# argumentcomputer/lurk-beta

Measured on AMD Instinct MI355X. Metric: MSM Mscalar-mul/s (Pallas Pedersen commitment, bases+scalars resident in HBM), higher is better.
Workload: dtype u32x8 (255-bit Montgomery, integer VALU)

## Files before the change

### lurk_beta_amd/csrc/common.hpp

```cpp
#pragma once
#include <hip/hip_runtime.h>

#include <cstdint>
#include <cstdio>
#include <cstring>
#include <condition_variable>
#include <functional>
#include <map>
#include <mutex>
#include <string>
#include <thread>
#include <utility>
#include <vector>

#include "../../include/lurk_hip.h"

namespace lurk {

void set_error(int code, const std::string& msg);
int last_error_code();

struct HipFailure {
    int code;
    std::string msg;
};

#define LURK_HIP_CHECK(expr)                                                                              \
    do {                                                                                                  \
        hipError_t _e = (expr);                                                                           \
        if (_e != hipSuccess) {                                                                           \
            (void)hipGetLastError();  \
            throw ::lurk::HipFailure{_e == hipErrorOutOfMemory ? LURK_HIP_ERR_OOM : LURK_HIP_ERR_HIP,     \
                                     std::string(#expr) + ": " + hipGetErrorString(_e)};                 \
        }                                                                                                 \
    } while (0)

#define LURK_REQUIRE(cond, msg)                                                       \
    do {                                                                              \
        if (!(cond)) throw ::lurk::HipFailure{LURK_HIP_ERR_INVALID_ARG, std::string(msg)}; \
    } while (0)

void require_device();

struct DeviceGuard {
    int prev = -1;
    bool switched = false;
    explicit DeviceGuard(int dev) {
        LURK_HIP_CHECK(hipGetDevice(&prev));
        if (prev != dev) {
            LURK_HIP_CHECK(hipSetDevice(dev));
            switched = true;
        }
    }
    ~DeviceGuard() {
        if (switched) (void)hipSetDevice(prev);
    }
    DeviceGuard(const DeviceGuard&) = delete;
    DeviceGuard& operator=(const DeviceGuard&) = delete;
};
int current_device();

void allow_dynamic_lds(const void* kernel, int bytes);

template <class F>
int host_guarded(F&& f) {
    try {
        f();
        set_error(0, "");
        return 0;
    } catch (const HipFailure& e) {
        set_error(e.code, e.msg);
        return e.code;
    } catch (const std::exception& e) {
        set_error(LURK_HIP_ERR_HIP, e.what());
        return LURK_HIP_ERR_HIP;
    }
}
template <class F>
int guarded(F&& f) {
    return host_guarded([&] {
        require_device();
        f();
    });
}
inline void nested_ok(int rc) {
    if (rc != 0) throw HipFailure{rc, lurk_hip_last_error()};
}

struct DevBuf {
    void* p = nullptr;
    size_t bytes = 0;
    DevBuf() = default;
    explicit DevBuf(size_t n) { alloc(n); }
    DevBuf(const DevBuf&) = delete;
    DevBuf& operator=(const DevBuf&) = delete;
    DevBuf(DevBuf&& o) noexcept : p(o.p), bytes(o.bytes) { o.p = nullptr; o.bytes = 0; }
    DevBuf& operator=(DevBuf&& o) noexcept {
        if (this != &o) { release(); p = o.p; bytes = o.bytes; o.p = nullptr; o.bytes = 0; }
        return *this;
    }
    ~DevBuf() { release(); }
    void alloc(size_t n) {
        release();
        if (n == 0) n = 16;
        LURK_HIP_CHECK(hipMalloc(&p, n));
        bytes = n;
    }
    void ensure(size_t n) {
        if (n > bytes) alloc(n);
    }
    void release() {
        if (p) (void)hipFree(p);
        p = nullptr;
        bytes = 0;
    }
    template <class T>
    T* as() const { return reinterpret_cast<T*>(p); }
};

class Profiler {
  public:
    static Profiler& get();
    void enable(bool on) { enabled_ = on; }
    bool enabled() const { return enabled_; }
    void reset();
    hipEvent_t begin(hipStream_t s);
    void end(const char* name, hipEvent_t a, hipStream_t s);
    void query(const char* prefix, double* total_ms, uint64_t* launches);

  private:
    struct Rec { std::string name; hipEvent_t a, b; int device; hipStream_t s; };
    std::mutex mu_;
    bool enabled_ = false;
    std::vector<Rec> recs_;
    std::map<int, std::vector<hipEvent_t>> pool_;
    std::map<std::string, std::pair<double, uint64_t>> done_;
    hipEvent_t get_event(int device);
    void dump_timeline();
};

struct ProfScope {
    hipStream_t s;
    const char* name;
    hipEvent_t a = nullptr;
    ProfScope(const char* nm, hipStream_t st) : s(st), name(nm) {
        if (Profiler::get().enabled()) a = Profiler::get().begin(s);
    }
    ~ProfScope() {
        if (a) Profiler::get().end(name, a, s);
    }
};

class DeviceWorker {
  public:
    explicit DeviceWorker(int device);
    ~DeviceWorker();
    void post(std::function<void()> job);
    void wait();
    int device() const { return device_; }

  private:
    void loop();
    int device_;
    std::mutex mu_;
    std::condition_variable cv_;
    std::function<void()> job_;
    bool has_job_ = false, busy_ = false, stop_ = false, failed_ = false;
    HipFailure err_{0, ""};
    std::thread th_;
};

struct MsmTableView {
    const void* table = nullptr;
    size_t npoints = 0;
    int curve = 0, window_bits = 0, windows = 1, form = 0, device = 0;
};
MsmTableView msm_ctx_table_view(const lurk_hip_msm_ctx* ctx);
int msm_multi_curve(const lurk_hip_msm_multi* key);
void msm_ctx_wait_pair_xyzz(lurk_hip_msm_ctx* ctx, int slot, void* out_lo_xyzz128, void* out_hi_xyzz128);
struct FoldedKeyLease {
    lurk_hip_msm_ctx* ctx = nullptr;
    bool owned = false;
    std::unique_lock<std::mutex> lk;
    FoldedKeyLease() = default;
    FoldedKeyLease(FoldedKeyLease&& o) noexcept : ctx(o.ctx), owned(o.owned), lk(std::move(o.lk)) {
        o.ctx = nullptr;
        o.owned = false;
    }
    FoldedKeyLease(const FoldedKeyLease&) = delete;
    ~FoldedKeyLease();
};
FoldedKeyLease msm_ctx_folded_child(lurk_hip_msm_ctx* parent, const void* d_points, size_t m, hipStream_t s);
void msm_ctx_drop_folded_child(const lurk_hip_msm_ctx* parent);

class ScratchArena {
  public:
    static ScratchArena& of(hipStream_t s);
    static size_t trim_all();
    void* push(size_t bytes);
    void pop(void* p);
    std::recursive_mutex mu;

  private:
    struct Block { char* base; size_t cap, top; };
    struct Live { void* p; size_t block, prev_top; bool freed; };
    std::vector<Block> blocks_;
    std::vector<Live> live_;
    size_t cur_ = 0;
};
struct ArenaBuf {
    ScratchArena* arena;
    void* p = nullptr;
    ArenaBuf(size_t bytes, hipStream_t s) : arena(&ScratchArena::of(s)) {
        arena->mu.lock();
        try {
            p = arena->push(bytes ? bytes : 32);
        } catch (...) {
            arena->mu.unlock();
            throw;
        }
    }
    ~ArenaBuf() {
        arena->pop(p);
        arena->mu.unlock();
    }
    ArenaBuf(const ArenaBuf&) = delete;
    ArenaBuf& operator=(const ArenaBuf&) = delete;
};

struct PoseidonImageView {
    const void* img = nullptr;
    int vec4 = 0, rf = 0, rp = 0;
};
PoseidonImageView poseidon_image_view(int field_id, int arity, hipStream_t s);

inline const char* curve_name(int curve) {
    switch (curve) {
        case LURK_CURVE_PALLAS: return "Pallas";
        case LURK_CURVE_VESTA: return "Vesta";
        case LURK_CURVE_BN254: return "BN254";
        case LURK_CURVE_GRUMPKIN: return "Grumpkin";
    }
    return "unknown";
}
inline void require_pasta_curve(int curve, const char* what) {
    if (curve == LURK_CURVE_PALLAS || curve == LURK_CURVE_VESTA) return;
    if (curve == LURK_CURVE_BN254 || curve == LURK_CURVE_GRUMPKIN)
        throw HipFailure{LURK_HIP_ERR_INVALID_ARG, std::string(what) + " is not offered on " + curve_name(curve) + " (Pallas and Vesta only)"};
    throw HipFailure{LURK_HIP_ERR_INVALID_ARG, "unknown curve id"};
}

inline unsigned div_up(size_t a, size_t b) { return (unsigned)((a + b - 1) / b); }

int num_cus();
unsigned grid_cap(unsigned per_cu);
void stream_pool_retain();

}
```

### lurk_beta_amd/csrc/curve29.cuh

```cuda
#pragma once
#include "curve.cuh"
#include "field29.cuh"

#ifndef LURK_ACC_Y3_ROW
#define LURK_ACC_Y3_ROW 1
#endif
#ifndef LURK_ACC_AFFINE_FIRST
#define LURK_ACC_AFFINE_FIRST 1
#endif
#ifndef LURK_F29_RARE_ATTR
#define LURK_F29_RARE_ATTR __attribute__((noinline))
#endif

namespace lurk {

template <class P>
LURK_HD F29<P> f29_carry_signed(const int32_t* t) {
    F29<P> r;
    int32_t c = 0;
#pragma unroll
    for (int i = 0; i < 8; i++) {
        int32_t x = t[i] + c;
        r.l[i] = (uint32_t)x & F29_MASK;
        c = x >> 29;
    }
    r.l[8] = (uint32_t)(t[8] + c);
    return r;
}


template <class P>
LURK_HD F29<P> f29_reduce_pasta(const F29<P>& v) {
    const uint32_t k = v.l[8] >> 22;
    const uint32_t km1 = k ? k - 1 : 0;
    int32_t t[9];
    uint64_t c = 0;
#pragma unroll
    for (int i = 0; i < 5; i++) {
        c += (uint64_t)km1 * f29_mod<P>(i);
        t[i] = (int32_t)v.l[i] - (int32_t)((uint32_t)c & F29_MASK);
        c >>= 29;
    }
    t[5] = (int32_t)v.l[5] - (int32_t)(uint32_t)c;
    t[6] = (int32_t)v.l[6];
    t[7] = (int32_t)v.l[7];
    t[8] = (int32_t)(v.l[8] & ((1u << 22) - 1u)) + (k ? (int32_t)(1u << 22) : 0);
    return f29_carry_signed<P>(t);
}
template <class P>
LURK_HD F29<P> f29_reduce_general(const F29<P>& v) {
    constexpr uint32_t D = (P::mod(7) >> 8) + 1u;
    static_assert(D > (1u << 21) && D <= (1u << 22), "f29_reduce_general: the modulus must have 253 or 254 bits");
    constexpr uint64_t mu = ((uint64_t)1 << 53) / D;
    F29_ASSERT(v.l[8] < (1u << 31), "f29_reduce: top limb >= 2^31");
    const uint32_t q = (uint32_t)(((uint64_t)v.l[8] * mu) >> 53);
    int32_t t[9];
    uint64_t c = 0;
#pragma unroll
    for (int i = 0; i < 8; i++) {
        c += (uint64_t)q * f29_mod<P>(i);
        t[i] = (int32_t)v.l[i] - (int32_t)((uint32_t)c & F29_MASK);
        c >>= 29;
    }
    c += (uint64_t)q * f29_mod<P>(8);
    t[8] = (int32_t)v.l[8] - (int32_t)(uint32_t)c;
    const F29<P> r = f29_carry_signed<P>(t);
    F29_ASSERT(r.l[8] < (1u << 24), "f29_reduce: result not below 2^256");
    return r;
}
template <class P>
LURK_HD F29<P> f29_reduce(const F29<P>& v) {
    if constexpr (f29_pasta_shape<P>()) return f29_reduce_pasta<P>(v);
    else return f29_reduce_general<P>(v);
}

template <class P>
struct Xyzz29 {
    F29<P> x, y, zz, zzz;
};

template <class P>
LURK_HD Xyzz<P> xyzz29_to_xyzz(const Xyzz29<P>& a, bool is_identity) {
    if (is_identity) return xyzz_identity<P>();
    Xyzz<P> r;
    r.x = f29_to_mont256<P>(a.x);
    r.y = f29_to_mont256<P>(a.y);
    r.zz = f29_to_mont256<P>(a.zz);
    r.zzz = f29_to_mont256<P>(a.zzz);
    return r;
}
template <class P>
LURK_HD void xyzz29_from_xyzz(const Xyzz<P>& a, Xyzz29<P>& r, bool& is_identity) {
    is_identity = xyzz_is_identity<P>(a);
    r.x = f29_from_mont256<P>(a.x);
    r.y = f29_from_mont256<P>(a.y);
    r.zz = f29_from_mont256<P>(a.zz);
    r.zzz = f29_from_mont256<P>(a.zzz);
}

template <class P>
LURK_HD uint32_t f29_multiple_candidate(const F29<P>& v) {
    if constexpr (f29_pasta_shape<P>()) return v.l[0];
    else return (v.l[0] * ((0u - f29_inv<P>()) & F29_MASK)) & F29_MASK;
}
template <class P>
LURK_HD bool f29_maybe_multiple_of_p(const F29<P>& v) {
    return f29_multiple_candidate<P>(v) < (f29_pasta_shape<P>() ? 128u : 256u);
}
template <class P>
LURK_HD bool f29_is_multiple_of_p(const F29<P>& v) {
    const uint32_t k = f29_multiple_candidate<P>(v);
    uint64_t c = 0;
    bool eq = true;
#pragma unroll
    for (int i = 0; i < 8; i++) {
        c += (uint64_t)k * f29_mod<P>(i);
        eq = eq && (v.l[i] == ((uint32_t)c & F29_MASK));
        c >>= 29;
    }
    c += (uint64_t)k * f29_mod<P>(8);
    return eq && (uint64_t)v.l[8] == c;
}

template <class P>
LURK_HD LURK_F29_RARE_ATTR Xyzz29<P> xyzz29_double_affine(F29<P> qx, F29<P> qy_signed) {
    const F29<P> u = f29_dbl<P>(qy_signed);
    const F29<P> v = f29_mul<P>(u, u);
    const F29<P> w = f29_mul30<P>(u, v);
    const F29<P> s = f29_mul30<P>(qx, v);
    const F29<P> xx = f29_sqr30<P>(qx);
    const F29<P> m = f29_carry<P>(f29_add<P>(f29_dbl<P>(xx), xx));
    const F29<P> m2 = f29_sqr30<P>(m);
    Xyzz29<P> r;
    r.x = f29_reduce<P>(f29_carry<P>(f29_sub<P>(m2, f29_dbl<P>(s))));
    const F29<P> t1 = f29_mul<P>(m, f29_sub<P>(s, r.x));
    const F29<P> t2 = f29_mul30<P>(w, qy_signed);
    r.y = f29_reduce<P>(f29_carry<P>(f29_sub<P>(t1, t2)));
    r.zz = v;
    r.zzz = w;
    return r;
}

template <class P, bool ACC_AFFINE = false>
LURK_HD void xyzz29_madd(Xyzz29<P>& acc, bool& acc_id, const Affine<P>& q, bool negate) {
    if (affine_is_identity<P>(q)) return;
    const F29<P> qx = f29_from_mont256<P>(q.x);
    const F29<P> qy = f29_from_mont256<P>(q.y);
    if (acc_id) {
        acc.x = qx;
        acc.y = negate ? f29_reduce<P>(f29_carry<P>(f29_sub<P>(f29_zero<P>(), qy))) : qy;
        Fe<P> one = fe_one<P>();
        acc.zz = f29_from_mont256<P>(one);
        acc.zzz = acc.zz;
        acc_id = false;
        return;
    }
    F29_ASSERT_LIMBS(acc.x, 29, "acc.x"); F29_ASSERT_TOP(acc.x, 27, "acc.x");
    F29_ASSERT_LIMBS(acc.y, 29, "acc.y"); F29_ASSERT_TOP(acc.y, 27, "acc.y");
    F29_ASSERT_LIMBS(acc.zz, 29, "acc.zz"); F29_ASSERT_TOP(acc.zz, 27, "acc.zz");
    F29_ASSERT_LIMBS(acc.zzz, 29, "acc.zzz"); F29_ASSERT_TOP(acc.zzz, 27, "acc.zzz");
    const F29<P> u2 = ACC_AFFINE ? qx : f29_mul30<P>(qx, acc.zz);
    const F29<P> s2 = ACC_AFFINE ? qy : f29_mul30<P>(qy, acc.zzz);
    const F29<P> p = f29_carry<P>(f29_sub<P>(u2, acc.x));
    F29<P> r;
#pragma unroll
    for (int i = 0; i < 9; i++) {
        F29_ASSERT(f29_bias<P>(i) >= acc.y.l[i], "madd: Y1 limb above the bias");
        r.l[i] = s2.l[i] + (negate ? acc.y.l[i] : f29_bias<P>(i) - acc.y.l[i]);
    }
    r = f29_carry<P>(r);
    if (f29_maybe_multiple_of_p<P>(p) && f29_is_multiple_of_p<P>(p)) {
        if (f29_maybe_multiple_of_p<P>(r) && f29_is_multiple_of_p<P>(r)) {
            const F29<P> qys = negate ? f29_reduce<P>(f29_carry<P>(f29_sub<P>(f29_zero<P>(), qy))) : qy;
            acc = xyzz29_double_affine<P>(qx, qys);
        } else {
            acc_id = true;
        }
        return;
    }
    const F29<P> pp = f29_sqr30<P>(p);
    const F29<P> ppp = f29_mul30<P>(p, pp);
    const F29<P> qq = f29_mul30<P>(acc.x, pp);
    const F29<P> r2 = f29_sqr30<P>(r);
    F29<P> x3 = f29_sub<P>(f29_sub<P>(r2, ppp), f29_dbl<P>(qq));
    x3 = f29_reduce<P>(f29_carry<P>(x3));
    F29<P> d;
#pragma unroll
    for (int i = 0; i < 9; i++) {
        F29_ASSERT(f29_bias<P>(i) >= qq.l[i] && f29_bias<P>(i) >= x3.l[i], "madd: Q / X3 limb above the bias");
        d.l[i] = negate ? x3.l[i] + (f29_bias<P>(i) - qq.l[i]) : qq.l[i] + (f29_bias<P>(i) - x3.l[i]);
    }
#if LURK_ACC_Y3_ROW
    Dot29<P> row;
    dot29_init<P>(row);
    dot29_mac<P>(row, r, f29_carry<P>(d));
    dot29_mac<P>(row, f29_carry<P>(f29_sub<P>(f29_zero<P>(), acc.y)), ppp);
    F29<P> y3 = f29_reduce<P>(dot29_finish2<P>(row));
#else
    const F29<P> t1 = f29_mul<P>(r, d);
    const F29<P> t2 = f29_mul30<P>(acc.y, ppp);
    F29<P> y3 = f29_reduce<P>(f29_carry<P>(f29_sub<P>(t1, t2)));
#endif
    acc.x = x3;
    acc.y = y3;
    if (ACC_AFFINE) {
        acc.zz = f29_reduce<P>(pp);
        acc.zzz = f29_reduce<P>(ppp);
    } else {
        acc.zz = f29_mul30<P>(acc.zz, pp);
        acc.zzz = f29_mul30<P>(acc.zzz, ppp);
    }
}

#ifndef LURK_ACC_SIGNED
#define LURK_ACC_SIGNED 1
#endif
#if F29_CHECKS_ACTIVE
#define F29S_ASSERT_ACC(v, what)                                                                                                  \
    do {                                                                                                                          \
        F29_ASSERT_LIMBS8(v, what);                                                                                               \
        const int32_t _t = (int32_t)(v).l[8];                                                                                     \
        if (_t < -(1 << 27) || _t >= (1 << 27)) { printf("F29 bound violated: %s top limb = %d (|value| >= 2^259)\n", what, _t); abort(); } \
    } while (0)
#define F29_ASSERT_LIMBS8(v, what)                                                                                                \
    do {                                                                                                                          \
        for (int _i = 0; _i < 8; _i++)                                                                                            \
            if ((v).l[_i] >> 29) { printf("F29 bound violated: %s limb %d = %u (>= 2^29)\n", what, _i, (v).l[_i]); abort(); }    \
    } while (0)
#else
#define F29S_ASSERT_ACC(v, what) ((void)0)
#define F29_ASSERT_LIMBS8(v, what) ((void)0)
#endif
template <class P>
LURK_HD F29<P> f29_sub_s(const F29<P>& a, const F29<P>& b) {
    F29<P> r;
#pragma unroll
    for (int i = 0; i < 9; i++) r.l[i] = a.l[i] - b.l[i];
    return r;
}
template <class P>
LURK_HD F29<P> f29_neg_s(const F29<P>& a) {
    F29<P> r;
#pragma unroll
    for (int i = 0; i < 9; i++) r.l[i] = 0u - a.l[i];
    return r;
}
template <class P>
LURK_HD F29<P> f29_carry_s(const F29<P>& a) {
    F29<P> r;
    uint32_t c = 0;
#pragma unroll
    for (int i = 0; i < 8; i++) {
        const uint32_t x = a.l[i] + c;
        r.l[i] = x & F29_MASK;
        c = (uint32_t)((int32_t)x >> 29);
    }
    r.l[8] = a.l[8] + c;
    return r;
}
template <class P>
LURK_HD F29<P> f29_norm_s(const F29<P>& a) {
    F29<P> t;
#pragma unroll
    for (int i = 0; i < 9; i++) t.l[i] = a.l[i] + f29_bias<P>(i);
    const F29<P> u = f29_carry<P>(t);
    F29_ASSERT(u.l[8] < (1u << 29), "f29_norm_s: |value| >= 2^260");
    return f29_reduce<P>(u);
}
template <class P>
LURK_HD bool f29_maybe_multiple_of_p_s(const F29<P>& v) {
    return ((v.l[0] + 64u) & F29_MASK) < 128u;
}
template <class P>
LURK_HD bool f29_is_multiple_of_p_s(const F29<P>& v) {
    F29<P> t;
#pragma unroll
    for (int i = 0; i < 9; i++) t.l[i] = v.l[i] + f29_bias<P>(i);
    t = f29_carry<P>(t);
    F29_ASSERT(t.l[8] < (1u << 29), "f29_is_multiple_of_p_s: |v| >= 64p");
    return f29_is_multiple_of_p<P>(t);
}

template <class P, bool ACC_AFFINE = false>
LURK_HD void xyzz29_madd_s(Xyzz29<P>& acc, bool& acc_id, const Affine<P>& q, bool negate) {
    if (affine_is_identity<P>(q)) return;
    const F29<P> qx = f29_from_mont256<P>(q.x);
    const F29<P> qy = f29_from_mont256<P>(q.y);
    const F29<P> qys = negate ? f29_neg_s<P>(qy) : qy;
    if (acc_id) {
        acc.x = qx;
        acc.y = negate ? f29_carry_s<P>(qys) : qy;
        Fe<P> one = fe_one<P>();
        acc.zz = f29_from_mont256<P>(one);
        acc.zzz = acc.zz;
        acc_id = false;
        return;
    }
    F29S_ASSERT_ACC(acc.x, "acc.x"); F29S_ASSERT_ACC(acc.y, "acc.y"); F29S_ASSERT_ACC(acc.zz, "acc.zz"); F29S_ASSERT_ACC(acc.zzz, "acc.zzz");
    const F29<P> u2 = ACC_AFFINE ? qx : f29_mul_s<P>(qx, acc.zz);
    const F29<P> s2 = ACC_AFFINE ? qys : f29_mul_s<P>(qys, acc.zzz);
    const F29<P> p = f29_sub_s<P>(u2, acc.x);
    const F29<P> r = ACC_AFFINE ? f29_carry_s<P>(f29_sub_s<P>(s2, acc.y)) : f29_sub_s<P>(s2, acc.y);
    if (f29_maybe_multiple_of_p_s<P>(p) && f29_is_multiple_of_p_s<P>(p)) {
        if (f29_maybe_multiple_of_p_s<P>(r) && f29_is_multiple_of_p_s<P>(r)) {
            const F29<P> qyn = negate ? f29_reduce<P>(f29_carry<P>(f29_sub<P>(f29_zero<P>(), qy))) : qy;
            acc = xyzz29_double_affine<P>(qx, qyn);
            acc.zz = f29_reduce<P>(acc.zz);
        } else {
            acc_id = true;
        }
        return;
    }
    const F29<P> pp = f29_sqr_s<P>(p);
    const F29<P> ppp = f29_mul_s<P>(p, pp);
    const F29<P> qq = f29_mul_s<P>(acc.x, pp);
    const F29<P> r2 = f29_sqr_s<P>(r);
    F29<P> x3;
#pragma unroll
    for (int i = 0; i < 9; i++) x3.l[i] = r2.l[i] - ppp.l[i] - (qq.l[i] << 1);
    x3 = f29_carry_s<P>(x3);
    const F29<P> d = f29_sub_s<P>(qq, x3);
    F29<P> y3 = dot29_row2_s<P>(r, d, f29_neg_s<P>(acc.y), ppp);
    if (ACC_AFFINE) {
        acc.x = f29_norm_s<P>(x3);
        acc.y = f29_norm_s<P>(y3);
        acc.zz = f29_reduce<P>(pp);
        acc.zzz = f29_norm_s<P>(ppp);
    } else {
        acc.x = x3;
        acc.y = y3;
        acc.zz = f29_mul_s<P>(acc.zz, pp);
        acc.zzz = f29_mul_s<P>(acc.zzz, ppp);
    }
    F29S_ASSERT_ACC(acc.x, "acc.x out"); F29S_ASSERT_ACC(acc.y, "acc.y out"); F29S_ASSERT_ACC(acc.zz, "acc.zz out"); F29S_ASSERT_ACC(acc.zzz, "acc.zzz out");
}
template <class P>
LURK_HD void xyzz29_norm_s(Xyzz29<P>& acc) {
    acc.x = f29_norm_s<P>(acc.x);
    acc.y = f29_norm_s<P>(acc.y);
    acc.zz = f29_norm_s<P>(acc.zz);
    acc.zzz = f29_norm_s<P>(acc.zzz);
}

template <class P>
LURK_HD Xyzz29<P> xyzz29_dbl(const Xyzz29<P>& a) {
    const F29<P> u = f29_dbl<P>(a.y);
    const F29<P> v = f29_mul<P>(u, u);
    const F29<P> w = f29_mul30<P>(u, v);
    const F29<P> s = f29_mul30<P>(a.x, v);
    const F29<P> xx = f29_sqr30<P>(a.x);
    const F29<P> m = f29_carry<P>(f29_add<P>(f29_dbl<P>(xx), xx));
    const F29<P> m2 = f29_sqr30<P>(m);
    Xyzz29<P> r;
    r.x = f29_reduce<P>(f29_carry<P>(f29_sub<P>(m2, f29_dbl<P>(s))));
    const F29<P> t1 = f29_mul<P>(m, f29_sub<P>(s, r.x));
    const F29<P> t2 = f29_mul30<P>(w, a.y);
    r.y = f29_reduce<P>(f29_carry<P>(f29_sub<P>(t1, t2)));
    r.zz = f29_mul30<P>(v, a.zz);
    r.zzz = f29_mul30<P>(w, a.zzz);
    return r;
}

template <class P>
LURK_HD LURK_F29_RARE_ATTR Xyzz29<P> xyzz29_double_general(Xyzz29<P> a) {
    const Xyzz<P> d = xyzz_dbl<P>(xyzz29_to_xyzz<P>(a, false));
    Xyzz29<P> r;
    bool id;
    xyzz29_from_xyzz<P>(d, r, id);
    return r;
}

template <class P>
LURK_HD void xyzz29_add(Xyzz29<P>& acc, bool& acc_id, const Xyzz29<P>& q, bool q_id) {
    if (q_id) return;
    if (acc_id) {
        acc = q;
        acc_id = false;
        return;
    }
    F29_ASSERT_LIMBS(acc.x, 29, "add acc.x"); F29_ASSERT_TOP(acc.x, 27, "add acc.x");
    F29_ASSERT_LIMBS(acc.y, 29, "add acc.y"); F29_ASSERT_TOP(acc.y, 27, "add acc.y");
    F29_ASSERT_LIMBS(acc.zz, 29, "add acc.zz"); F29_ASSERT_TOP(acc.zz, 27, "add acc.zz");
    F29_ASSERT_LIMBS(acc.zzz, 29, "add acc.zzz"); F29_ASSERT_TOP(acc.zzz, 27, "add acc.zzz");
    F29_ASSERT_LIMBS(q.x, 29, "add q.x"); F29_ASSERT_TOP(q.x, 27, "add q.x");
    F29_ASSERT_LIMBS(q.y, 29, "add q.y"); F29_ASSERT_TOP(q.y, 27, "add q.y");
    F29_ASSERT_LIMBS(q.zz, 29, "add q.zz"); F29_ASSERT_TOP(q.zz, 27, "add q.zz");
    F29_ASSERT_LIMBS(q.zzz, 29, "add q.zzz"); F29_ASSERT_TOP(q.zzz, 27, "add q.zzz");
    const F29<P> u1 = f29_mul30<P>(acc.x, q.zz);
    const F29<P> u2 = f29_mul30<P>(q.x, acc.zz);
    const F29<P> s1 = f29_mul30<P>(acc.y, q.zzz);
    const F29<P> s2 = f29_mul30<P>(q.y, acc.zzz);
    const F29<P> p = f29_carry<P>(f29_sub<P>(u2, u1));
    const F29<P> r = f29_carry<P>(f29_sub<P>(s2, s1));
    if (f29_maybe_multiple_of_p<P>(p) && f29_is_multiple_of_p<P>(p)) {
        if (f29_maybe_multiple_of_p<P>(r) && f29_is_multiple_of_p<P>(r)) acc = xyzz29_double_general<P>(acc);
        else acc_id = true;
        return;
    }
    const F29<P> pp = f29_sqr30<P>(p);
    const F29<P> ppp = f29_mul30<P>(p, pp);
    const F29<P> qq = f29_mul30<P>(u1, pp);
    const F29<P> r2 = f29_sqr30<P>(r);
    F29<P> x3 = f29_sub<P>(f29_sub<P>(r2, ppp), f29_dbl<P>(qq));
    x3 = f29_reduce<P>(f29_carry<P>(x3));
    F29<P> d;
#pragma unroll
    for (int i = 0; i < 9; i++) {
        F29_ASSERT(f29_bias<P>(i) >= x3.l[i], "add: X3 limb above the bias");
        d.l[i] = qq.l[i] + (f29_bias<P>(i) - x3.l[i]);
    }
    Dot29<P> row;
    dot29_init<P>(row);
    dot29_mac<P>(row, r, f29_carry<P>(d));
    dot29_mac<P>(row, f29_carry<P>(f29_sub<P>(f29_zero<P>(), s1)), ppp);
    const F29<P> y3 = f29_reduce<P>(dot29_finish2<P>(row));
    const F29<P> zz12 = f29_mul30<P>(acc.zz, q.zz);
    const F29<P> zzz12 = f29_mul30<P>(acc.zzz, q.zzz);
    acc.x = x3;
    acc.y = y3;
    acc.zz = f29_mul30<P>(zz12, pp);
    acc.zzz = f29_mul30<P>(zzz12, ppp);
}

template <class P>
LURK_HD Xyzz<P> xyzz_sum_via29(const Xyzz<P>* pts, uint32_t nt) {
    if (nt == 0) return xyzz_identity<P>();
    if (nt == 1) return pts[0];
    Xyzz29<P> acc, q;
    bool acc_id, q_id;
    xyzz29_from_xyzz<P>(pts[0], acc, acc_id);
    for (uint32_t i = 1; i < nt; i++) {
        xyzz29_from_xyzz<P>(pts[i], q, q_id);
        xyzz29_add<P>(acc, acc_id, q, q_id);
    }
    return xyzz29_to_xyzz<P>(acc, acc_id);
}

template <class P>
struct Plane29 {
    Xyzz29<P> p;
    uint32_t id, pad[3];
};
template <class P>
LURK_HD void plane_load(const Plane29<P>* __restrict__ src, Xyzz29<P>& v, bool& id) {
    const Plane29<P> r = *src;
    v = r.p;
    id = r.id != 0;
}
template <class P>
LURK_HD void plane_store(Plane29<P>* __restrict__ dst, const Xyzz29<P>& v, bool id) {
    if (!id) {
        F29_ASSERT_LIMBS(v.x, 29, "record x"); F29_ASSERT_TOP(v.x, 27, "record x");
        F29_ASSERT_LIMBS(v.y, 29, "record y"); F29_ASSERT_TOP(v.y, 27, "record y");
        F29_ASSERT_LIMBS(v.zz, 29, "record zz"); F29_ASSERT_TOP(v.zz, 27, "record zz");
        F29_ASSERT_LIMBS(v.zzz, 29, "record zzz"); F29_ASSERT_TOP(v.zzz, 27, "record zzz");
    }
    Plane29<P> o;
    o.p = v;
    o.id = id;
    o.pad[0] = o.pad[1] = o.pad[2] = 0;
    *dst = o;
}
template <class P>
LURK_HD void plane_store_identity(Plane29<P>* __restrict__ dst) {
    Xyzz29<P> z;
    z.x = z.y = z.zz = z.zzz = f29_zero<P>();
    plane_store<P>(dst, z, true);
}
template <class P>
LURK_HD void plane_sum(const Plane29<P>* recs, uint32_t nt, Xyzz29<P>& acc, bool& acc_id) {
    plane_load<P>(recs, acc, acc_id);
    for (uint32_t i = 1; i < nt; i++) {
        Xyzz29<P> q;
        bool q_id;
        plane_load<P>(recs + i, q, q_id);
        xyzz29_add<P>(acc, acc_id, q, q_id);
    }
}

template <class P>
LURK_HD bool plane_finalize_bucket(Plane29<P>* records, uint32_t NB, size_t key, uint32_t nt, uint32_t first, uint32_t fin_small) {
    if (nt == 1) return false;
    if (nt == 0) {
        plane_store_identity<P>(records + key);
        return false;
    }
    if (nt > fin_small) return true;
    Xyzz29<P> acc;
    bool acc_id;
    plane_sum<P>(records + NB + first, nt, acc, acc_id);
    plane_store<P>(records + key, acc, acc_id);
    return false;
}

#if defined(__HIPCC__)
template <class P, int BLOCK>
__device__ __forceinline__ void block_tree_sum29(Xyzz29<P>& acc, bool& acc_id, Plane29<P>* sh) {
    const int t = threadIdx.x;
    plane_store<P>(sh + t, acc, acc_id);
    __syncthreads();
    for (int stride = BLOCK / 2; stride >= 1; stride >>= 1) {
        if (t < stride) {
            Xyzz29<P> q;
            bool q_id;
            plane_load<P>(sh + t + stride, q, q_id);
            xyzz29_add<P>(acc, acc_id, q, q_id);
            plane_store<P>(sh + t, acc, acc_id);
        }
        __syncthreads();
    }
}
#endif

typedef uint32_t Rec16 __attribute__((vector_size(16), may_alias));
struct Rec64 {
    Rec16 q[4];
};
template <class P>
LURK_HD Rec64 rec64_load(const Affine<P>* table, uint32_t e) {
    static_assert(sizeof(Affine<P>) == 64 && alignof(Affine<P>) >= 16, "a table record is four aligned 16-byte words");
    const Rec16* p = reinterpret_cast<const Rec16*>(table + (e & 0x7fffffffu));
    Rec64 r;
#pragma unroll
    for (int i = 0; i < 4; i++) r.q[i] = p[i];
    return r;
}
template <class P>
LURK_HD Affine<P> rec64_affine(const Rec64& r) {
    Affine<P> a;
#pragma unroll
    for (int i = 0; i < 8; i++) {
        a.x.l[i] = r.q[i >> 2][i & 3];
        a.y.l[i] = r.q[2 + (i >> 2)][i & 3];
    }
    return a;
}
template <class P>
LURK_HD Affine<P> msm_task_next29(const uint32_t* sorted, const Affine<P>* table, uint32_t j, uint32_t last, bool& neg_next, uint32_t& e_ahead,
                                  Rec64& rec, bool& negate) {
    const Affine<P> q = rec64_affine<P>(rec);
    negate = neg_next;
    neg_next = (e_ahead & 0x80000000u) != 0;
    rec = rec64_load<P>(table, e_ahead);
    e_ahead = sorted[j + 2 < last ? j + 2 : j];
    return q;
}

template <class P>
LURK_HD constexpr bool msm_acc_signed() {
    return LURK_ACC_SIGNED != 0 && f29_p1_form<P>();
}
template <class P, bool ACC_AFFINE = false>
LURK_HD void xyzz29_madd_task(Xyzz29<P>& acc, bool& acc_id, const Affine<P>& q, bool negate) {
    if constexpr (msm_acc_signed<P>()) xyzz29_madd_s<P, ACC_AFFINE>(acc, acc_id, q, negate);
    else xyzz29_madd<P, ACC_AFFINE>(acc, acc_id, q, negate);
}
template <class P, bool PIPELINED = false>
LURK_HD void msm_task_accumulate29_loop(const uint32_t* sorted, uint32_t first, uint32_t last, const Affine<P>* table, Xyzz29<P>& acc, bool& acc_id) {
    acc.x = acc.y = acc.zz = acc.zzz = f29_zero<P>();
    acc_id = true;
    if (PIPELINED) {
        if (first >= last) return;
        const uint32_t e_first = sorted[first];
        bool neg_next = (e_first & 0x80000000u) != 0;
        Rec64 rec = rec64_load<P>(table, e_first);
        uint32_t e_ahead = sorted[first + 1 < last ? first + 1 : first];
        uint32_t j = first;
        bool negate;
#if LURK_ACC_AFFINE_FIRST
        {
            const Affine<P> q = msm_task_next29<P>(sorted, table, j, last, neg_next, e_ahead, rec, negate);
            xyzz29_madd_task<P>(acc, acc_id, q, negate);
            j++;
        }
        if (j < last) {
            const Affine<P> q = msm_task_next29<P>(sorted, table, j, last, neg_next, e_ahead, rec, negate);
            if (!acc_id) xyzz29_madd_task<P, true>(acc, acc_id, q, negate);
            else xyzz29_madd_task<P>(acc, acc_id, q, negate);
            j++;
        }
#endif
        for (; j < last; j++) {
            const Affine<P> q = msm_task_next29<P>(sorted, table, j, last, neg_next, e_ahead, rec, negate);
            xyzz29_madd_task<P>(acc, acc_id, q, negate);
        }
        return;
    }
#if LURK_ACC_AFFINE_FIRST
    uint32_t j = first;
    if (j < last) {
        const uint32_t e = sorted[j++];
        xyzz29_madd_task<P>(acc, acc_id, table[e & 0x7fffffffu], (e & 0x80000000u) != 0);
    }
    if (j < last) {
        const uint32_t e = sorted[j++];
        const Affine<P> q = table[e & 0x7fffffffu];
#if LURK_ACC_AFFINE_FIRST
        if (!acc_id) xyzz29_madd_task<P, true>(acc, acc_id, q, (e & 0x80000000u) != 0);
        else
#endif
            xyzz29_madd_task<P>(acc, acc_id, q, (e & 0x80000000u) != 0);
    }
    for (; j < last; j++) {
        const uint32_t e = sorted[j];
        const Affine<P> q = table[e & 0x7fffffffu];
        xyzz29_madd_task<P>(acc, acc_id, q, (e & 0x80000000u) != 0);
    }
#else
    for (uint32_t j = first; j < last; j++) {
        const uint32_t e = sorted[j];
#ifdef LURK_ACC_DEBUG_TABLE_MASK
        const Affine<P> q = table[e & LURK_ACC_DEBUG_TABLE_MASK];
#else
        const Affine<P> q = table[e & 0x7fffffffu];
#endif
        xyzz29_madd_task<P>(acc, acc_id, q, (e & 0x80000000u) != 0);
    }
#endif
}
template <class P, bool PIPELINED = false>
LURK_HD void msm_task_accumulate29_raw(const uint32_t* sorted, uint32_t first, uint32_t last, const Affine<P>* table, Xyzz29<P>& acc, bool& acc_id) {
    msm_task_accumulate29_loop<P, PIPELINED>(sorted, first, last, table, acc, acc_id);
    if constexpr (msm_acc_signed<P>()) {
        if (!acc_id) xyzz29_norm_s<P>(acc);
    }
}
template <class P, bool PIPELINED = false>
LURK_HD Xyzz<P> msm_task_accumulate29(const uint32_t* sorted, uint32_t first, uint32_t last, const Affine<P>* table) {
    Xyzz29<P> acc;
    bool acc_id;
    msm_task_accumulate29_raw<P, PIPELINED>(sorted, first, last, table, acc, acc_id);
    return xyzz29_to_xyzz<P>(acc, acc_id);
}

}
```

### lurk_beta_amd/csrc/field.cuh

```cuda
#pragma once
#include <stdint.h>

#if defined(__HIPCC__)
#define LURK_HD __host__ __device__ __forceinline__
#else
#define LURK_HD inline
#endif

namespace lurk {

struct PallasFp {
    static constexpr int ID = 0;
    static constexpr int NBITS = 255;
    static constexpr uint32_t INV = 0xffffffffu;
    LURK_HD static constexpr uint32_t mod(int i) {
        constexpr uint32_t m[8] = {0x00000001u, 0x992d30edu, 0x094cf91bu, 0x224698fcu, 0x00000000u, 0x00000000u, 0x00000000u, 0x40000000u};
        return m[i];
    }
    LURK_HD static constexpr uint32_t r(int i) {
        constexpr uint32_t m[8] = {0xfffffffdu, 0x34786d38u, 0xe41914adu, 0x992c350bu, 0xffffffffu, 0xffffffffu, 0xffffffffu, 0x3fffffffu};
        return m[i];
    }
    LURK_HD static constexpr uint32_t r2(int i) {
        constexpr uint32_t m[8] = {0x0000000fu, 0x8c78ecb3u, 0x8b0de0e7u, 0xd7d30dbdu, 0xc3c95d18u, 0x7797a99bu, 0x7b9cb714u, 0x096d41afu};
        return m[i];
    }
    LURK_HD static constexpr uint32_t w32(int i) {
        constexpr uint32_t m[8] = {0xbad6dbf0u, 0xa28db849u, 0xd3b539dfu, 0x9083cd03u, 0x9dc8448eu, 0xfba6b9cau, 0x7b89c6dau, 0x3ec92874u};
        return m[i];
    }
};

struct PallasFq {
    static constexpr int ID = 1;
    static constexpr int NBITS = 255;
    static constexpr uint32_t INV = 0xffffffffu;
    LURK_HD static constexpr uint32_t mod(int i) {
        constexpr uint32_t m[8] = {0x00000001u, 0x8c46eb21u, 0x0994a8ddu, 0x224698fcu, 0x00000000u, 0x00000000u, 0x00000000u, 0x40000000u};
        return m[i];
    }
    LURK_HD static constexpr uint32_t r(int i) {
        constexpr uint32_t m[8] = {0xfffffffdu, 0x5b2b3e9cu, 0xe3420567u, 0x992c350bu, 0xffffffffu, 0xffffffffu, 0xffffffffu, 0x3fffffffu};
        return m[i];
    }
    LURK_HD static constexpr uint32_t r2(int i) {
        constexpr uint32_t m[8] = {0x0000000fu, 0xfc9678ffu, 0x891a16e3u, 0x67bb433du, 0x04ccf590u, 0x7fae2310u, 0x7ccfdaa9u, 0x096d41afu};
        return m[i];
    }
    LURK_HD static constexpr uint32_t w32(int i) {
        constexpr uint32_t m[8] = {0x8c9942deu, 0x21807742u, 0x21b60494u, 0xcc495789u, 0xb2efbee2u, 0xac2e5d27u, 0x7f2db056u, 0x0b79fa89u};
        return m[i];
    }
};

struct Bn254Fr {
    static constexpr int ID = 2;
    static constexpr int NBITS = 254;
    static constexpr uint32_t INV = 0xefffffffu;
    LURK_HD static constexpr uint32_t mod(int i) {
        constexpr uint32_t m[8] = {0xf0000001u, 0x43e1f593u, 0x79b97091u, 0x2833e848u, 0x8181585du, 0xb85045b6u, 0xe131a029u, 0x30644e72u};
        return m[i];
    }
    LURK_HD static constexpr uint32_t r(int i) {
        constexpr uint32_t m[8] = {0x4ffffffbu, 0xac96341cu, 0x9f60cd29u, 0x36fc7695u, 0x7879462eu, 0x666ea36fu, 0x9a07df2fu, 0x0e0a77c1u};
        return m[i];
    }
    LURK_HD static constexpr uint32_t r2(int i) {
        constexpr uint32_t m[8] = {0xae216da7u, 0x1bb8e645u, 0xe35c59e3u, 0x53fe3ab1u, 0x53bb8085u, 0x8c49833du, 0x7f4e44a5u, 0x0216d0b1u};
        return m[i];
    }
    LURK_HD static constexpr uint32_t w32(int i) { return 0; }
};

struct Bn254Fq {
    static constexpr int ID = 3;
    static constexpr int NBITS = 254;
    static constexpr uint32_t INV = 0xe4866389u;
    LURK_HD static constexpr uint32_t mod(int i) {
        constexpr uint32_t m[8] = {0xd87cfd47u, 0x3c208c16u, 0x6871ca8du, 0x97816a91u, 0x8181585du, 0xb85045b6u, 0xe131a029u, 0x30644e72u};
        return m[i];
    }
    LURK_HD static constexpr uint32_t r(int i) {
        constexpr uint32_t m[8] = {0xc58f0d9du, 0xd35d438du, 0xf5c70b3du, 0x0a78eb28u, 0x7879462cu, 0x666ea36fu, 0x9a07df2fu, 0x0e0a77c1u};
        return m[i];
    }
    LURK_HD static constexpr uint32_t r2(int i) {
        constexpr uint32_t m[8] = {0x538afa89u, 0xf32cfc5bu, 0xd44501fbu, 0xb5e71911u, 0x0a417ff6u, 0x47ab1effu, 0xcab8351fu, 0x06d89f71u};
        return m[i];
    }
    LURK_HD static constexpr uint32_t w32(int i) { return 0; }
};

template <class P>
struct alignas(16) Fe {
    uint32_t l[8];
};

template <class P>
LURK_HD Fe<P> fe_zero() {
    Fe<P> z;
#pragma unroll
    for (int i = 0; i < 8; i++) z.l[i] = 0;
    return z;
}
template <class P>
LURK_HD Fe<P> fe_one() {
    Fe<P> z;
#pragma unroll
    for (int i = 0; i < 8; i++) z.l[i] = P::r(i);
    return z;
}
template <class P>
LURK_HD Fe<P> fe_r2() {
    Fe<P> z;
#pragma unroll
    for (int i = 0; i < 8; i++) z.l[i] = P::r2(i);
    return z;
}
template <class P>
LURK_HD bool fe_is_zero(const Fe<P>& a) {
    uint32_t o = 0;
#pragma unroll
    for (int i = 0; i < 8; i++) o |= a.l[i];
    return o == 0;
}
template <class P>
LURK_HD bool fe_eq(const Fe<P>& a, const Fe<P>& b) {
    uint32_t o = 0;
#pragma unroll
    for (int i = 0; i < 8; i++) o |= a.l[i] ^ b.l[i];
    return o == 0;
}

LURK_HD uint32_t addc32(uint32_t a, uint32_t b, uint32_t& carry) {
#if defined(__HIP_DEVICE_COMPILE__)
    unsigned c;
    uint32_t r = __builtin_addc(a, b, carry, &c);
    carry = c;
    return r;
#else
    uint64_t x = (uint64_t)a + b + carry;
    carry = (uint32_t)(x >> 32);
    return (uint32_t)x;
#endif
}
LURK_HD uint32_t subb32(uint32_t a, uint32_t b, uint32_t& borrow) {
#if defined(__HIP_DEVICE_COMPILE__)
    unsigned c;
    uint32_t r = __builtin_subc(a, b, borrow, &c);
    borrow = c;
    return r;
#else
    uint64_t x = (uint64_t)a - b - borrow;
    borrow = (uint32_t)(x >> 63);
    return (uint32_t)x;
#endif
}

#if defined(LURK_FE_CHECK) && !defined(__HIP_DEVICE_COMPILE__)
#define FE_CHECKS_ACTIVE 1
}
#include <cstdio>
#include <cstdlib>
namespace lurk {
template <class P>
inline void fe_assert_canonical(const uint32_t* v, const char* what) {
    for (int i = 7; i >= 0; i--) {
        if (v[i] < P::mod(i)) return;
        if (v[i] > P::mod(i)) break;
    }
    fprintf(stderr, "Fe contract violated: %s operand >= p\n", what);
    abort();
}
#define FE_ASSERT_CANONICAL(P, x, what) fe_assert_canonical<P>((x).l, what)
#else
#define FE_CHECKS_ACTIVE 0
#define FE_ASSERT_CANONICAL(P, x, what) ((void)0)
#endif

template <class P>
LURK_HD void fe_cond_sub(uint32_t* t) {
    uint32_t d[8];
    uint32_t borrow = 0;
#pragma unroll
    for (int i = 0; i < 8; i++) d[i] = subb32(t[i], P::mod(i), borrow);
#pragma unroll
    for (int i = 0; i < 8; i++) t[i] = borrow ? t[i] : d[i];
}

template <class P>
LURK_HD Fe<P> fe_add(const Fe<P>& a, const Fe<P>& b) {
    FE_ASSERT_CANONICAL(P, a, "fe_add");
    FE_ASSERT_CANONICAL(P, b, "fe_add");
    Fe<P> r;
    uint32_t c = 0;
#pragma unroll
    for (int i = 0; i < 8; i++) r.l[i] = addc32(a.l[i], b.l[i], c);
    fe_cond_sub<P>(r.l);
    return r;
}
template <class P>
LURK_HD Fe<P> fe_sub(const Fe<P>& a, const Fe<P>& b) {
    FE_ASSERT_CANONICAL(P, a, "fe_sub");
    FE_ASSERT_CANONICAL(P, b, "fe_sub");
    Fe<P> r;
    uint32_t borrow = 0;
#pragma unroll
    for (int i = 0; i < 8; i++) r.l[i] = subb32(a.l[i], b.l[i], borrow);
    uint32_t mask = 0u - borrow, c = 0;
#pragma unroll
    for (int i = 0; i < 8; i++) r.l[i] = addc32(r.l[i], P::mod(i) & mask, c);
    return r;
}
template <class P>
LURK_HD Fe<P> fe_neg(const Fe<P>& a) {
    return fe_sub<P>(fe_zero<P>(), a);
}
template <class P>
LURK_HD Fe<P> fe_dbl(const Fe<P>& a) {
    return fe_add<P>(a, a);
}

template <class P>
LURK_HD Fe<P> fe_mul_cios(const Fe<P>& a, const Fe<P>& b) {
    uint32_t t[8];
#pragma unroll
    for (int i = 0; i < 8; i++) t[i] = 0;
#pragma unroll
    for (int i = 0; i < 8; i++) {
        uint32_t bi = b.l[i];
        uint64_t acc = (uint64_t)a.l[0] * bi + t[0];
        uint32_t m = (uint32_t)acc * P::INV;
        uint64_t red = (uint64_t)m * P::mod(0) + (uint32_t)acc;
        uint32_t c1 = (uint32_t)(acc >> 32), c2 = (uint32_t)(red >> 32);
#pragma unroll
        for (int j = 1; j < 8; j++) {
            acc = (uint64_t)a.l[j] * bi + t[j] + c1;
            c1 = (uint32_t)(acc >> 32);
            red = (uint64_t)m * P::mod(j) + (uint32_t)acc + c2;
            c2 = (uint32_t)(red >> 32);
            t[j - 1] = (uint32_t)red;
        }
        t[7] = c1 + c2;
    }
    fe_cond_sub<P>(t);
    Fe<P> r;
#pragma unroll
    for (int i = 0; i < 8; i++) r.l[i] = t[i];
    return r;
}

LURK_HD void mad_c(uint64_t& acc, uint64_t& carry, uint32_t a, uint32_t b) {
#if defined(__HIP_DEVICE_COMPILE__)
    asm volatile("v_mad_u64_u32 %0, %1, %2, %3, %0" : "+v"(acc), "=s"(carry) : "v"(a), "v"(b));
#else
    uint64_t p = (uint64_t)a * b;
    acc += p;
    carry = (acc < p) ? 1u : 0u;
#endif
}
LURK_HD void mad_ck(uint64_t& acc, uint64_t& carry, uint32_t a, uint32_t k) {
#if defined(__HIP_DEVICE_COMPILE__)
    asm volatile("v_mad_u64_u32 %0, %1, %2, %3, %0" : "+v"(acc), "=s"(carry) : "v"(a), "s"(k));
#else
    mad_c(acc, carry, a, k);
#endif
}
LURK_HD void column_fence() {
#if defined(__HIP_DEVICE_COMPILE__)
    asm volatile("s_nop 1");
#endif
}
LURK_HD void fold_carry(uint32_t& hi, uint64_t carry) {
#if defined(__HIP_DEVICE_COMPILE__)
    asm volatile("v_addc_co_u32_e64 %0, vcc, 0, %0, %1" : "+v"(hi) : "s"(carry) : "vcc");
#else
    hi += (uint32_t)carry;
#endif
}

template <class P>
LURK_HD Fe<P> fe_mul_fips(const Fe<P>& a, const Fe<P>& b) {
    uint32_t m[8], t[8];
    uint64_t lo = 0;
    uint32_t hi = 0;
#pragma unroll
    for (int k = 0; k < 16; k++) {
        uint64_t cm[16];
        int n = 0;
        const int i0 = k < 8 ? 0 : k - 7, i1 = k < 8 ? k : 7;
#pragma unroll
        for (int i = i0; i <= i1; i++) mad_c(lo, cm[n++], a.l[i], b.l[k - i]);
#pragma unroll
        for (int i = i0; i <= (k < 8 ? k - 1 : 7); i++)
            if (P::mod(k - i) != 0) mad_ck(lo, cm[n++], m[i], P::mod(k - i));
        bool carry_in_one = false;
        uint32_t c0 = 0;
        if (k < 8) {
            c0 = (uint32_t)lo;
            m[k] = c0 * P::INV;
            if (P::mod(0) == 1 && P::INV == 0xffffffffu) {
                carry_in_one = true;
            } else {
                mad_ck(lo, cm[n++], m[k], P::mod(0));
            }
        }
        column_fence();
#pragma unroll
        for (int i = 0; i < n; i++) fold_carry(hi, cm[i]);
        if (k >= 8) t[k - 8] = (uint32_t)lo;
        lo = (lo >> 32) | ((uint64_t)hi << 32);
        if (carry_in_one) lo += (c0 != 0 ? 1u : 0u);
        hi = 0;
    }
    fe_cond_sub<P>(t);
    Fe<P> r;
#pragma unroll
    for (int i = 0; i < 8; i++) r.l[i] = t[i];
    return r;
}

#if !defined(__HIP_DEVICE_COMPILE__) && defined(__SIZEOF_INT128__)
template <class P>
inline Fe<P> fe_mul_host64(const Fe<P>& a, const Fe<P>& b) {
    typedef unsigned __int128 u128;
    uint64_t x[4], y[4], m[4], t[6] = {0, 0, 0, 0, 0, 0};
    for (int i = 0; i < 4; i++) {
        x[i] = (uint64_t)a.l[2 * i] | ((uint64_t)a.l[2 * i + 1] << 32);
        y[i] = (uint64_t)b.l[2 * i] | ((uint64_t)b.l[2 * i + 1] << 32);
        m[i] = (uint64_t)P::mod(2 * i) | ((uint64_t)P::mod(2 * i + 1) << 32);
    }
    uint64_t inv32 = P::INV;
    uint64_t ninv = (uint64_t)0 - inv32;
    ninv *= 2 - m[0] * ninv;
    const uint64_t inv = (uint64_t)0 - ninv;
    for (int i = 0; i < 4; i++) {
        u128 c = 0;
        for (int j = 0; j < 4; j++) {
            c += (u128)x[j] * y[i] + t[j];
            t[j] = (uint64_t)c;
            c >>= 64;
        }
        c += t[4];
        t[4] = (uint64_t)c;
        t[5] = (uint64_t)(c >> 64);
        uint64_t q = t[0] * inv;
        c = ((u128)q * m[0] + t[0]) >> 64;
        for (int j = 1; j < 4; j++) {
            c += (u128)q * m[j] + t[j];
            t[j - 1] = (uint64_t)c;
            c >>= 64;
        }
        c += t[4];
        t[3] = (uint64_t)c;
        t[4] = t[5] + (uint64_t)(c >> 64);
    }
    uint64_t d[4];
    u128 br = 0;
    for (int i = 0; i < 4; i++) {
        u128 v = (u128)t[i] - m[i] - br;
        d[i] = (uint64_t)v;
        br = (v >> 64) & 1;
    }
    bool ge = t[4] != 0 || br == 0;
    Fe<P> r;
    for (int i = 0; i < 4; i++) {
        uint64_t v = ge ? d[i] : t[i];
        r.l[2 * i] = (uint32_t)v;
        r.l[2 * i + 1] = (uint32_t)(v >> 32);
    }
    return r;
}
#define LURK_HAVE_HOST64 1
#endif

#ifndef LURK_MUL_IMPL
#define LURK_MUL_IMPL 2
#endif
}
#include "field_mul_asm.cuh"
#include "field_mul_asm_bn254fq.cuh"
namespace lurk {
template <class P>
LURK_HD Fe<P> fe_mul_inline(const Fe<P>& a, const Fe<P>& b) {
#if LURK_MUL_IMPL == 0
    return fe_mul_cios<P>(a, b);
#elif LURK_MUL_IMPL == 2 && defined(__HIP_DEVICE_COMPILE__)
    return fe_mul_asm<P>(a, b);
#elif !defined(__HIP_DEVICE_COMPILE__) && defined(LURK_HAVE_HOST64) && !defined(LURK_HOST_PORTABLE_MUL)
    return fe_mul_host64<P>(a, b);
#else
    return fe_mul_fips<P>(a, b);
#endif
}
#if defined(__HIPCC__)
template <class P>
__device__ __attribute__((noinline)) Fe<P> fe_mul_call(Fe<P> a, Fe<P> b) {
    return fe_mul_inline<P>(a, b);
}
#endif
template <class P>
LURK_HD Fe<P> fe_mul(const Fe<P>& a, const Fe<P>& b) {
    FE_ASSERT_CANONICAL(P, a, "fe_mul");
    FE_ASSERT_CANONICAL(P, b, "fe_mul");
#if defined(__HIP_DEVICE_COMPILE__) && !defined(LURK_MUL_FORCE_INLINE)
    return fe_mul_call<P>(a, b);
#else
    return fe_mul_inline<P>(a, b);
#endif
}
template <class P>
LURK_HD void fe_cond_sub2(uint32_t* t) {
    uint32_t d[8];
    uint32_t borrow = 0;
#pragma unroll
    for (int i = 0; i < 8; i++) {
        uint32_t twop = (P::mod(i) << 1) | (i ? (P::mod(i - 1) >> 31) : 0u);
        d[i] = subb32(t[i], twop, borrow);
    }
#pragma unroll
    for (int i = 0; i < 8; i++) t[i] = borrow ? t[i] : d[i];
}

template <class P>
struct DotAcc {
    uint64_t col[15];
    uint32_t h[15];
};
template <class P>
LURK_HD void dot_init(DotAcc<P>& A) {
#pragma unroll
    for (int k = 0; k < 15; k++) {
        A.col[k] = 0;
        A.h[k] = 0;
    }
}
template <class P>
LURK_HD void dot_mac(DotAcc<P>& A, const Fe<P>& a, const Fe<P>& b) {
#pragma unroll
    for (int j = 0; j < 8; j++) {
        uint64_t cm[8];
#pragma unroll
        for (int l = 0; l < 8; l++) mad_c(A.col[j + l], cm[l], a.l[j], b.l[l]);
        column_fence();
#pragma unroll
        for (int l = 0; l < 8; l++) fold_carry(A.h[j + l], cm[l]);
    }
}
template <class P>
LURK_HD void fe_redc16_portable(uint32_t* t, const uint32_t* vin) {
    uint32_t v[17];
#pragma unroll
    for (int i = 0; i < 16; i++) v[i] = vin[i];
    v[16] = 0;
#pragma unroll
    for (int k = 0; k < 8; k++) {
        uint32_t m = v[k] * P::INV;
        uint64_t c = 0;
#pragma unroll
        for (int j = 0; j < 8; j++) {
            uint64_t x = (uint64_t)m * P::mod(j) + v[k + j] + c;
            v[k + j] = (uint32_t)x;
            c = x >> 32;
        }
#pragma unroll
        for (int j = k + 8; j < 17; j++) {
            uint64_t x = (uint64_t)v[j] + c;
            v[j] = (uint32_t)x;
            c = x >> 32;
        }
    }
#pragma unroll
    for (int i = 0; i < 8; i++) t[i] = v[8 + i];
}

template <class P, int T>
LURK_HD Fe<P> dot_finish(const DotAcc<P>& A) {
    uint32_t x[16], v[16];
    uint32_t c1 = 0, c2 = 0;
#pragma unroll
    for (int k = 0; k < 16; k++) {
        uint32_t lo = k < 15 ? (uint32_t)A.col[k] : 0u;
        uint32_t hi = k >= 1 ? (uint32_t)(A.col[k - 1] >> 32) : 0u;
        x[k] = addc32(lo, hi, c1);
    }
#pragma unroll
    for (int k = 0; k < 16; k++) v[k] = addc32(x[k], k >= 2 ? A.h[k - 2] : 0u, c2);
    uint32_t t[8];
#if defined(__HIP_DEVICE_COMPILE__) && LURK_MUL_IMPL == 2
    fe_redc16_asm<P>(t, v);
#else
    fe_redc16_portable<P>(t, v);
#endif
    if (T > 3) fe_cond_sub2<P>(t);
    fe_cond_sub<P>(t);
    Fe<P> r;
#pragma unroll
    for (int i = 0; i < 8; i++) r.l[i] = t[i];
    return r;
}

template <class P>
LURK_HD Fe<P> fe_sqr(const Fe<P>& a) {
    return fe_mul<P>(a, a);
}

template <class P>
LURK_HD Fe<P> fe_to_mont(const Fe<P>& a) {
    return fe_mul<P>(a, fe_r2<P>());
}
template <class P>
LURK_HD Fe<P> fe_from_mont(const Fe<P>& a) {
    Fe<P> one = fe_zero<P>();
    one.l[0] = 1;
    return fe_mul<P>(a, one);
}
template <class P>
LURK_HD Fe<P> fe_from_u64(uint64_t v) {
    Fe<P> x = fe_zero<P>();
    x.l[0] = (uint32_t)v;
    x.l[1] = (uint32_t)(v >> 32);
    return fe_to_mont<P>(x);
}

template <class P>
LURK_HD Fe<P> fe_pow(const Fe<P>& a, const uint32_t* e) {
    Fe<P> acc = fe_one<P>();
    for (int i = 255; i >= 0; i--) {
        acc = fe_sqr<P>(acc);
        if ((e[i >> 5] >> (i & 31)) & 1) acc = fe_mul<P>(acc, a);
    }
    return acc;
}
#if !defined(__HIP_DEVICE_COMPILE__)
namespace host_inv {
struct U256 {
    uint64_t w[4];
};
inline bool is_one(const U256& a) { return a.w[0] == 1 && (a.w[1] | a.w[2] | a.w[3]) == 0; }
inline bool ge(const U256& a, const U256& b) {
    for (int i = 3; i >= 0; i--)
        if (a.w[i] != b.w[i]) return a.w[i] > b.w[i];
    return true;
}
inline uint64_t add(U256& a, const U256& b) {
    unsigned __int128 c = 0;
    for (int i = 0; i < 4; i++) {
        c += (unsigned __int128)a.w[i] + b.w[i];
        a.w[i] = (uint64_t)c;
        c >>= 64;
    }
    return (uint64_t)c;
}
inline void sub(U256& a, const U256& b) {
    uint64_t borrow = 0;
    for (int i = 0; i < 4; i++) {
        const uint64_t bi = b.w[i], t = a.w[i] - bi, t2 = t - borrow;
        borrow = (uint64_t)(a.w[i] < bi) | (uint64_t)(t < borrow);
        a.w[i] = t2;
    }
}
inline void shr1(U256& a, uint64_t top) {
    a.w[0] = (a.w[0] >> 1) | (a.w[1] << 63);
    a.w[1] = (a.w[1] >> 1) | (a.w[2] << 63);
    a.w[2] = (a.w[2] >> 1) | (a.w[3] << 63);
    a.w[3] = (a.w[3] >> 1) | (top << 63);
}
inline void halve_mod(U256& x, const U256& p) {
    if (x.w[0] & 1) {
        const uint64_t c = add(x, p);
        shr1(x, c);
    } else {
        shr1(x, 0);
    }
}
inline void sub_mod(U256& x, const U256& y, const U256& p) {
    if (ge(x, y)) {
        sub(x, y);
    } else {
        U256 t = p;
        sub(t, y);
        add(x, t);
    }
}
inline bool is_zero(const U256& a) { return (a.w[0] | a.w[1] | a.w[2] | a.w[3]) == 0; }
inline U256 inverse(U256 u, const U256& p) {
    while (ge(u, p)) sub(u, p);
    if (is_zero(u)) return u;
    U256 v = p, x1 = {{1, 0, 0, 0}}, x2 = {{0, 0, 0, 0}};
    while (!is_one(u) && !is_one(v)) {
        while (!(u.w[0] & 1)) {
            shr1(u, 0);
            halve_mod(x1, p);
        }
        while (!(v.w[0] & 1)) {
            shr1(v, 0);
            halve_mod(x2, p);
        }
        if (ge(u, v)) {
            sub(u, v);
            sub_mod(x1, x2, p);
        } else {
            sub(v, u);
            sub_mod(x2, x1, p);
        }
    }
    return is_one(u) ? x1 : x2;
}
}
#endif

template <class P>
LURK_HD Fe<P> fe_inv(const Fe<P>& a) {
#if !defined(__HIP_DEVICE_COMPILE__)
    host_inv::U256 u, p;
    for (int i = 0; i < 4; i++) {
        u.w[i] = (uint64_t)a.l[2 * i] | ((uint64_t)a.l[2 * i + 1] << 32);
        p.w[i] = (uint64_t)P::mod(2 * i) | ((uint64_t)P::mod(2 * i + 1) << 32);
    }
    const host_inv::U256 x = host_inv::inverse(u, p);
    Fe<P> xi;
    for (int i = 0; i < 4; i++) {
        xi.l[2 * i] = (uint32_t)x.w[i];
        xi.l[2 * i + 1] = (uint32_t)(x.w[i] >> 32);
    }
    const Fe<P> r2 = fe_r2<P>();
    return fe_mul<P>(xi, fe_mul<P>(r2, r2));
#else
    uint32_t e[8];
    uint32_t borrow = 2;
    for (int i = 0; i < 8; i++) {
        uint64_t x = (uint64_t)P::mod(i) - borrow;
        e[i] = (uint32_t)x;
        borrow = (uint32_t)(x >> 63);
    }
    return fe_pow<P>(a, e);
#endif
}
template <class P>
LURK_HD Fe<P> fe_inv_pow(const Fe<P>& a) {
    uint32_t e[8];
    uint32_t borrow = 2;
    for (int i = 0; i < 8; i++) {
        uint64_t x = (uint64_t)P::mod(i) - borrow;
        e[i] = (uint32_t)x;
        borrow = (uint32_t)(x >> 63);
    }
    return fe_pow<P>(a, e);
}

template <class P>
LURK_HD bool fe_canonical_ge_mod(const uint32_t* v) {
    for (int i = 7; i >= 0; i--) {
        if (v[i] > P::mod(i)) return true;
        if (v[i] < P::mod(i)) return false;
    }
    return true;
}

}
```

### lurk_beta_amd/csrc/msm_batch.hip

```cpp
#include "msm_batch.hpp"

#include "msm_ctx.hpp"
#include "msm_launch_plan.hpp"
#include "msm_sort.hpp"
#include "msm_stages.hpp"

namespace lurk {

constexpr int BATCH_BLOCK = 1024;
constexpr uint32_t BATCH_BINS_MAX = 2048;
constexpr int BATCH_SCAN_BLOCK = 1024;
static_assert(MSM_BATCH_GRP == (uint32_t)MSM_GRP && MSM_BATCH_TASK_TARGET == MSM_TASK_TARGET, "msm_batch_plan.hpp restates the plan stage's constants");
constexpr uint32_t BATCH_LEN_HIST_WORDS = 2 * (MSM_S_MAX + 1);
static_assert(BATCH_LEN_HIST_WORDS <= BATCH_SCAN_BLOCK, "one lane per word");

template <class F>
__device__ __forceinline__ void msm_batch_walk(const uint32_t (&s)[8], int c, int h, int W, uint32_t B, uint32_t j, uint32_t stride, F&& f) {
    uint32_t r[8];
#pragma unroll
    for (int t = 0; t < 8; t++) r[t] = s[t];
    uint32_t carry = 0;
    for (int w = 0; w < W; w++) {
        const uint32_t d = msm_digit_next(r, c, carry);
        const uint32_t mag = d & ~MSM_SIGN;
        if (!mag) continue;
        uint32_t lo, hi;
        msm_batch_split(mag, h, lo, hi);
        const uint32_t entry = ((uint32_t)w * stride + j) | (d & MSM_SIGN);
        if (lo) f(lo - 1u, entry);
        if (hi) f(B + hi - 1u, entry);
    }
}

template <class SF, bool SCATTER>
__global__ __launch_bounds__(BATCH_BLOCK) void msm_batch_emit_kernel(const uint4* __restrict__ scalars, MsmBatchSegs segs, uint32_t total, int c, int h, int W,
                                                                      uint32_t B, uint32_t stride, int is_mont, uint32_t* __restrict__ counters,
                                                                      uint32_t* __restrict__ sorted, uint32_t cap) {
    __builtin_amdgcn_s_setprio(3);
    __shared__ uint32_t hist[BATCH_BINS_MAX], run[BATCH_BINS_MAX];
    const uint32_t first = blockIdx.x * BATCH_BLOCK, i = first + threadIdx.x, bins = 2 * B;
    const uint32_t k0 = msm_batch_segment(segs.seg_start, segs.count, first);
    uint32_t* own = counters + (size_t)2 * k0 * B;
    for (uint32_t b = threadIdx.x; b < bins; b += BATCH_BLOCK) hist[b] = 0;
    __syncthreads();
    const bool live = i < total;
    uint32_t k = k0, j = 0, s8[8] = {0, 0, 0, 0, 0, 0, 0, 0};
    if (live) {
        k = msm_batch_segment(segs.seg_start, segs.count, i);
        j = i - segs.seg_start[k];
        const size_t at = (size_t)segs.off[k] + j;
        const uint4 lo4 = scalars[2 * at], hi4 = scalars[2 * at + 1];
        Fe<SF> s;
        s.l[0] = lo4.x; s.l[1] = lo4.y; s.l[2] = lo4.z; s.l[3] = lo4.w;
        s.l[4] = hi4.x; s.l[5] = hi4.y; s.l[6] = hi4.z; s.l[7] = hi4.w;
        if (is_mont) s = fe_from_mont<SF>(s);
#pragma unroll
        for (int t = 0; t < 8; t++) s8[t] = s.l[t];
    }
    const bool local = k == k0;
    uint32_t* mine = counters + (size_t)2 * k * B;
    if (live) {
        msm_batch_walk(s8, c, h, W, B, j, stride, [&](uint32_t bin, uint32_t) {
            if (local) atomicAdd(&hist[bin], 1u);
            else if (!SCATTER) atomicAdd(&mine[bin], 1u);
        });
    }
    __syncthreads();
    if (!SCATTER) {
        for (uint32_t b = threadIdx.x; b < bins; b += BATCH_BLOCK)
            if (hist[b]) atomicAdd(&own[b], hist[b]);
        return;
    }
    for (uint32_t b = threadIdx.x; b < bins; b += BATCH_BLOCK) {
        const uint32_t n = hist[b];
        run[b] = n ? atomicAdd(&own[b], n) : 0u;
        hist[b] = 0;
    }
    __syncthreads();
    if (live) {
        msm_batch_walk(s8, c, h, W, B, j, stride, [&](uint32_t bin, uint32_t entry) {
            const uint32_t pos = local ? run[bin] + atomicAdd(&hist[bin], 1u) : atomicAdd(&mine[bin], 1u);
            if (pos < cap) sorted[pos] = entry;
        });
    }
}

__global__ __launch_bounds__(BATCH_SCAN_BLOCK) void msm_batch_scan_kernel(const uint32_t* __restrict__ cnt, uint32_t* __restrict__ bucket_start,
                                                                           uint32_t* __restrict__ cursor, uint32_t NB, uint32_t* __restrict__ big_count,
                                                                           uint32_t* __restrict__ len_hist) {
    __builtin_amdgcn_s_setprio(3);
    __shared__ uint32_t part[BATCH_SCAN_BLOCK];
    const uint32_t t = threadIdx.x, per = (NB + BATCH_SCAN_BLOCK - 1) / BATCH_SCAN_BLOCK;
    const uint32_t lo = t * per < NB ? t * per : NB, hi = lo + per < NB ? lo + per : NB;
    uint32_t sum = 0;
    for (uint32_t b = lo; b < hi; b++) sum += cnt[b];
    part[t] = sum;
    __syncthreads();
    for (uint32_t off = 1; off < BATCH_SCAN_BLOCK; off <<= 1) {
        const uint32_t v = t >= off ? part[t - off] : 0u;
        __syncthreads();
        part[t] += v;
        __syncthreads();
    }
    uint32_t run = part[t] - sum;
    for (uint32_t b = lo; b < hi; b++) {
        bucket_start[b] = run;
        cursor[b] = run;
        run += cnt[b];
    }
    if (t == 0) *big_count = 0;
    if (t < BATCH_LEN_HIST_WORDS) len_hist[t] = 0;
}

void MsmBatchWork::ensure(const MsmBatchPlan& pl, size_t xyzz_bytes) {
    const size_t nb = pl.NBp;
    len_hist.ensure(BATCH_LEN_HIST_WORDS * 4);
    if (pl.planned) {
        task_start.ensure((size_t)pl.NG * (MSM_GRP + 1) * 4);
        group_tasks.ensure(64 * 4);
        group_task_base.ensure(64 * 4);
        task_info.ensure(pl.nt * sizeof(uint2));
        task_dest.ensure(pl.nt * 4);
        task_order.ensure(pl.nt * 4);
    }
    cnt.ensure(nb * 4);
    bucket_start.ensure(nb * 4);
    cursor.ensure(nb * 4);
    sorted.ensure(pl.max_entries * 4);
    records.ensure((nb + (pl.planned ? pl.nt : 0)) * MSM_RECORD_BYTES);
    big_list.ensure(nb * 4);
    big_count.ensure(16);
    planes_a.ensure(msm_reduce_plane_bytes(nb));
    planes_b.ensure(msm_reduce_plane_bytes(nb));
    const size_t need = (size_t)pl.G * (pl.h + 1) * xyzz_bytes;
    if (need > host_pts_bytes) {
        if (host_pts) (void)hipHostFree(host_pts);
        host_pts = nullptr;
        host_pts_bytes = 0;
        LURK_HIP_CHECK(hipHostMalloc(&host_pts, need));
        host_pts_bytes = need;
    }
}

template <class P, class SF>
void msm_batch_enqueue(MsmBatchWork& bw, const MsmBatchPlan& pl, const void* d_scalars, int is_mont, const Affine<P>* table, size_t stride, hipStream_t s) {
    LURK_REQUIRE(pl.total > 0 && pl.total <= LURK_MSM_BATCH_MAX_TOTAL && pl.NB <= MSM_DIRECT_MAX_BUCKETS && pl.NBp >= pl.NB && pl.NBp <= MSM_DIRECT_MAX_BUCKETS,
                 "batch: plan out of range");
    LURK_REQUIRE((size_t)pl.W * stride < ((size_t)1 << 31), "batch: table index out of range");
    LURK_REQUIRE(2 * pl.B <= BATCH_BINS_MAX, "batch: more bins per vector than the emit kernel's LDS holds");
    bw.ensure(pl, sizeof(Xyzz<P>));
    uint32_t *cnt = bw.cnt.as<uint32_t>(), *bucket_start = bw.bucket_start.as<uint32_t>(), *cursor = bw.cursor.as<uint32_t>(), *sorted = bw.sorted.as<uint32_t>();
    const dim3 grid(div_up(pl.total, BATCH_BLOCK)), block(BATCH_BLOCK);
    {
        ProfScope ps("msm_batch_sort", s);
        LURK_HIP_CHECK(hipMemsetAsync(cnt, 0, (size_t)pl.NBp * 4, s));
        hipLaunchKernelGGL((msm_batch_emit_kernel<SF, false>), grid, block, 0, s, (const uint4*)d_scalars, pl.segs, (uint32_t)pl.total, pl.c, pl.h, pl.W, pl.B,
                           (uint32_t)stride, is_mont, cnt, sorted, (uint32_t)pl.max_entries);
        hipLaunchKernelGGL(msm_batch_scan_kernel, dim3(1), dim3(BATCH_SCAN_BLOCK), 0, s, (const uint32_t*)cnt, bucket_start, cursor, pl.NBp,
                           bw.big_count.as<uint32_t>(), bw.len_hist.as<uint32_t>());
        hipLaunchKernelGGL((msm_batch_emit_kernel<SF, true>), grid, block, 0, s, (const uint4*)d_scalars, pl.segs, (uint32_t)pl.total, pl.c, pl.h, pl.W, pl.B,
                           (uint32_t)stride, is_mont, cursor, sorted, (uint32_t)pl.max_entries);
        LURK_HIP_CHECK(hipGetLastError());
    }
    Plane29<P>* records = (Plane29<P>*)bw.records.p;
    uint32_t *big_list = bw.big_list.as<uint32_t>(), *big_count = bw.big_count.as<uint32_t>();
    if (!pl.planned) {
        ProfScope ps("msm_batch_accumulate_direct", s);
        msm_launch_bucket_direct<P>(sorted, table, bucket_start, cnt, pl.NB, pl.max_entries, records, big_list, big_count, s);
    } else {
        uint32_t *task_start = bw.task_start.as<uint32_t>(), *group_task_base = bw.group_task_base.as<uint32_t>(), *task_dest = bw.task_dest.as<uint32_t>(),
                 *order = bw.task_order.as<uint32_t>();
        uint2* task_info = bw.task_info.as<uint2>();
        {
            ProfScope ps("msm_batch_tasks", s);
            msm_launch_plan_tasks(cnt, bucket_start, task_start, bw.group_tasks.as<uint32_t>(), group_task_base, pl.NG, pl.NBp, task_info, task_dest,
                                  bw.len_hist.as<uint32_t>(), order, pl.nt, (uint32_t)pl.S, 0, s);
        }
        {
            ProfScope ps("msm_batch_accumulate", s);
            msm_launch_accumulate<P>(sorted, table, task_info, order, task_dest, group_task_base, pl.NG, records, pl.nt, s);
        }
        {
            ProfScope ps("msm_batch_finalize", s);
            msm_launch_finalize<P>(records, cnt, task_start, group_task_base, pl.NBp, big_list, big_count, (uint32_t)pl.S, s);
            msm_launch_big_buckets<P>(records, cnt, task_start, group_task_base, pl.NBp, big_list, big_count, (uint32_t)pl.S, s);
        }
    }
    {
        ProfScope ps("msm_batch_reduce", s);
        msm_launch_reduce<P>(records, bw.planes_a.p, bw.planes_b.p, pl.h + 1, (int)pl.G, pl.B, (Xyzz<P>*)bw.host_pts, s);
    }
    LURK_HIP_CHECK(hipGetLastError());
}

template <class P>
Xyzz<P> msm_batch_host_point(const MsmBatchWork& bw, const MsmBatchPlan& pl, uint32_t k) {
    const int h = pl.h;
    const Xyzz<P>* v = (const Xyzz<P>*)bw.host_pts;
    const Xyzz<P>*lo = v + (size_t)(2 * k) * (h + 1), *hi = lo + (h + 1);
    Xyzz<P> acc = xyzz_identity<P>();
    for (int j = 2 * h - 1; j >= 0; j--) {
        acc = xyzz_dbl<P>(acc);
        if (j >= h) xyzz_add<P>(acc, hi[1 + (j - h)]);
        else xyzz_add<P>(acc, lo[1 + j]);
        if (j == h) xyzz_add<P>(acc, hi[0]);
    }
    xyzz_add<P>(acc, lo[0]);
    return acc;
}

#define LURK_BATCH_INSTANTIATE(P, SF)                                                                                                        \
    template void msm_batch_enqueue<P, SF>(MsmBatchWork&, const MsmBatchPlan&, const void*, int, const Affine<P>*, size_t, hipStream_t); \
    template Xyzz<P> msm_batch_host_point<P>(const MsmBatchWork&, const MsmBatchPlan&, uint32_t);
LURK_BATCH_INSTANTIATE(PallasFp, PallasFq)
LURK_BATCH_INSTANTIATE(PallasFq, PallasFp)
LURK_BATCH_INSTANTIATE(Bn254Fq, Bn254Fr)
LURK_BATCH_INSTANTIATE(Bn254Fr, Bn254Fq)

}

using namespace lurk;

extern "C" {

int lurk_hip_msm_ctx_submit_batch_dev(lurk_hip_msm_ctx* ctx, int slot, const void* d_scalars32, const size_t* offsets, const size_t* lens, size_t count, int is_mont,
                                      void* stream) {
    return guarded([&] {
        LURK_REQUIRE(ctx, "batch: null ctx");
        LURK_REQUIRE(offsets, "batch: null offsets");
        LURK_REQUIRE(lens, "batch: null lens");
        LURK_REQUIRE(count != 0, "batch: no vectors (count == 0)");
        LURK_REQUIRE(count <= LURK_MSM_BATCH_MAX_VECTORS, "batch: more than LURK_MSM_BATCH_MAX_VECTORS vectors");
        bool any = false;
        for (size_t k = 0; k < count; k++) any = any || lens[k] != 0;
        LURK_REQUIRE(!any || d_scalars32, "batch: null scalars");
        DeviceGuard dg(ctx->impl->device);
        ctx->impl->submit_batch(slot, d_scalars32, offsets, lens, count, is_mont, (hipStream_t)stream);
    });
}
int lurk_hip_msm_ctx_wait_batch(lurk_hip_msm_ctx* ctx, int slot, void* out_jacobian96) {
    return guarded([&] {
        LURK_REQUIRE(ctx, "batch: null ctx");
        LURK_REQUIRE(out_jacobian96, "batch: null output");
        DeviceGuard dg(ctx->impl->device);
        ctx->impl->wait_batch(slot, out_jacobian96);
    });
}

}
```

### lurk_beta_amd/csrc/msm_bucket_direct.hip

```cpp
#include "common.hpp"
#include "msm_core.cuh"
#include "curve29.cuh"
#include "msm_stages.hpp"

namespace lurk {

constexpr int DIRECT_BLOCK = 256;
constexpr uint32_t DIRECT_CAP = 64;

template <class P, int L>
__global__ __launch_bounds__(DIRECT_BLOCK) void msm_bucket_direct_kernel(const uint32_t* __restrict__ sorted, const Affine<P>* __restrict__ table,
                                                                           const uint32_t* __restrict__ bucket_start, const uint32_t* __restrict__ cnt,
                                                                           uint32_t NB, Plane29<P>* __restrict__ buckets, uint32_t* __restrict__ big_list,
                                                                           uint32_t* __restrict__ big_count) {
    __builtin_amdgcn_s_setprio(1);
    const size_t lane = (size_t)blockIdx.x * DIRECT_BLOCK + threadIdx.x;
    size_t key = lane / L;
    const uint32_t sub = (uint32_t)(lane % L);
    const bool live = key < NB;
    if (!live) key = NB - 1;
    uint32_t n = live ? cnt[key] : 0u;
    const uint32_t start = bucket_start[key];
    const bool big = n > (uint32_t)L * DIRECT_CAP;
    if (big) {
        if (sub == 0) big_list[atomicAdd(big_count, 1u)] = (uint32_t)key;
        n = 0;
    }
    const uint32_t per = (n + L - 1) / L;
    uint32_t first = start + sub * per, last = first + per;
    if (first > start + n) first = start + n;
    if (last > start + n) last = start + n;
    Xyzz29<P> acc;
    bool acc_id;
    msm_task_accumulate29_raw<P>(sorted, first, last, table, acc, acc_id);
#pragma unroll
    for (int off = L / 2; off >= 1; off >>= 1) {
        Xyzz29<P> o;
        bool o_id;
#pragma unroll
        for (int k = 0; k < 9; k++) {
            o.x.l[k] = __shfl_xor(acc.x.l[k], off);
            o.y.l[k] = __shfl_xor(acc.y.l[k], off);
            o.zz.l[k] = __shfl_xor(acc.zz.l[k], off);
            o.zzz.l[k] = __shfl_xor(acc.zzz.l[k], off);
        }
        o_id = __shfl_xor((int)acc_id, off) != 0;
        xyzz29_add<P>(acc, acc_id, o, o_id);
    }
    if (live && !big && sub == 0) plane_store<P>(buckets + key, acc, acc_id);
}

template <class P>
__global__ __launch_bounds__(DIRECT_BLOCK) void msm_bucket_direct_big_kernel(const uint32_t* __restrict__ sorted, const Affine<P>* __restrict__ table,
                                                                               const uint32_t* __restrict__ bucket_start, const uint32_t* __restrict__ cnt,
                                                                               Plane29<P>* __restrict__ buckets, const uint32_t* __restrict__ big_list,
                                                                               const uint32_t* __restrict__ big_count) {
    __builtin_amdgcn_s_setprio(1);
    extern __shared__ uint4 lds_raw[];
    Plane29<P>* sh = reinterpret_cast<Plane29<P>*>(lds_raw);
    const uint32_t nbig = *big_count;
    for (uint32_t i = blockIdx.x; i < nbig; i += gridDim.x) {
        const uint32_t key = big_list[i], n = cnt[key], start = bucket_start[key];
        Xyzz29<P> acc;
        acc.x = acc.y = acc.zz = acc.zzz = f29_zero<P>();
        bool acc_id = true;
        for (uint32_t j = threadIdx.x; j < n; j += DIRECT_BLOCK) {
            const uint32_t e = sorted[start + j];
            xyzz29_madd<P>(acc, acc_id, table[e & 0x7fffffffu], (e & 0x80000000u) != 0);
        }
        block_tree_sum29<P, DIRECT_BLOCK>(acc, acc_id, sh);
        if (threadIdx.x == 0) plane_store<P>(buckets + key, acc, acc_id);
        __syncthreads();
    }
}

#ifndef LURK_MSM_BN254_TU
int msm_bucket_direct_lanes(size_t NB, size_t entries) {
    int L = 1;
    while (L < 4 && NB * (size_t)(2 * L) <= 131072 && entries / (NB * (size_t)(2 * L)) >= 4) L *= 2;
    return L;
}
#endif

template <class P>
void msm_launch_bucket_direct(const uint32_t* sorted, const Affine<P>* table, const uint32_t* bucket_start, const uint32_t* cnt, uint32_t NB, size_t entries,
                              Plane29<P>* buckets, uint32_t* big_list, uint32_t* big_count, hipStream_t s) {
    const int L = msm_bucket_direct_lanes(NB, entries);
    const dim3 grid((unsigned)div_up((size_t)NB * L, DIRECT_BLOCK)), block(DIRECT_BLOCK);
    if (L == 1) hipLaunchKernelGGL((msm_bucket_direct_kernel<P, 1>), grid, block, 0, s, sorted, table, bucket_start, cnt, NB, buckets, big_list, big_count);
    else if (L == 2) hipLaunchKernelGGL((msm_bucket_direct_kernel<P, 2>), grid, block, 0, s, sorted, table, bucket_start, cnt, NB, buckets, big_list, big_count);
    else hipLaunchKernelGGL((msm_bucket_direct_kernel<P, 4>), grid, block, 0, s, sorted, table, bucket_start, cnt, NB, buckets, big_list, big_count);
    hipLaunchKernelGGL((msm_bucket_direct_big_kernel<P>), dim3(128), block, DIRECT_BLOCK * sizeof(Plane29<P>), s, sorted, table, bucket_start, cnt, buckets, big_list,
                       big_count);
}
#define LURK_DIRECT_INSTANTIATE(P)                                                                                                                      \
    template void msm_launch_bucket_direct<P>(const uint32_t*, const Affine<P>*, const uint32_t*, const uint32_t*, uint32_t, size_t, Plane29<P>*, uint32_t*, \
                                              uint32_t*, hipStream_t);
#ifdef LURK_MSM_BN254_TU
LURK_DIRECT_INSTANTIATE(Bn254Fq)
LURK_DIRECT_INSTANTIATE(Bn254Fr)
#else
LURK_DIRECT_INSTANTIATE(PallasFp)
LURK_DIRECT_INSTANTIATE(PallasFq)
#endif

}
```

### lurk_beta_amd/csrc/msm_finalize.hip

```cpp
#include "common.hpp"
#include "msm_core.cuh"
#include "curve29.cuh"
#include "msm_stages.hpp"

namespace lurk {

#ifndef LURK_FINALIZE_WAVES
#define LURK_FINALIZE_WAVES 4
#endif
#define LURK_FINALIZE_BOUNDS __launch_bounds__(256, LURK_FINALIZE_WAVES)
template <class P>
__global__ LURK_FINALIZE_BOUNDS void msm_finalize_kernel(Plane29<P>* records, const uint32_t* __restrict__ cnt, const uint32_t* __restrict__ task_start,
                                                             const uint32_t* __restrict__ group_task_base, uint32_t NB, uint32_t* __restrict__ big_list,
                                                             uint32_t* __restrict__ big_count, uint32_t S) {
    __builtin_amdgcn_s_setprio(3);
    const size_t key = (size_t)blockIdx.x * 256 + threadIdx.x;
    if (key >= NB) return;
    const uint32_t nt = (cnt[key] + S - 1) / S;
    uint32_t first = 0;
    if (nt >= 2 && nt <= MSM_FIN_SMALL) {
        const uint32_t g = (uint32_t)(key / MSM_GRP), b = (uint32_t)(key % MSM_GRP);
        first = group_task_base[g] + task_start[(size_t)g * (MSM_GRP + 1) + b];
    }
    if (plane_finalize_bucket<P>(records, NB, key, nt, first, MSM_FIN_SMALL)) big_list[atomicAdd(big_count, 1u)] = (uint32_t)key;
}

template <class P>
__global__ LURK_FINALIZE_BOUNDS void msm_big_bucket_kernel(Plane29<P>* records, const uint32_t* __restrict__ cnt, const uint32_t* __restrict__ task_start,
                                                               const uint32_t* __restrict__ group_task_base, uint32_t NB,
                                                               const uint32_t* __restrict__ big_list, const uint32_t* __restrict__ big_count, uint32_t S) {
    __builtin_amdgcn_s_setprio(3);
    extern __shared__ uint4 lds_raw[];
    Plane29<P>* sh = reinterpret_cast<Plane29<P>*>(lds_raw);
    const uint32_t nbig = *big_count;
    for (uint32_t i = blockIdx.x; i < nbig; i += gridDim.x) {
        const uint32_t key = big_list[i];
        const uint32_t g = key / MSM_GRP, b = key % MSM_GRP;
        const uint32_t nt = (cnt[key] + S - 1) / S;
        const Plane29<P>* tasks = records + NB + (group_task_base[g] + task_start[(size_t)g * (MSM_GRP + 1) + b]);
        Xyzz29<P> acc, q;
        acc.x = acc.y = acc.zz = acc.zzz = f29_zero<P>();
        bool acc_id = true, q_id;
        for (uint32_t j = threadIdx.x; j < nt; j += 256) {
            plane_load<P>(tasks + j, q, q_id);
            xyzz29_add<P>(acc, acc_id, q, q_id);
        }
        block_tree_sum29<P, 256>(acc, acc_id, sh);
        if (threadIdx.x == 0) plane_store<P>(records + key, acc, acc_id);
        __syncthreads();
    }
}

template <class P>
void msm_launch_finalize(Plane29<P>* records, const uint32_t* cnt, const uint32_t* task_start, const uint32_t* group_task_base, uint32_t NB,
                         uint32_t* big_list, uint32_t* big_count, uint32_t S, hipStream_t s) {
    static_assert(sizeof(Plane29<P>) == MSM_RECORD_BYTES, "the slot's record array is sized by MSM_RECORD_BYTES");
    hipLaunchKernelGGL((msm_finalize_kernel<P>), dim3(div_up((size_t)NB, 256)), dim3(256), 0, s, records, cnt, task_start, group_task_base, NB, big_list, big_count,
                       S);
}
template <class P>
void msm_launch_big_buckets(Plane29<P>* records, const uint32_t* cnt, const uint32_t* task_start, const uint32_t* group_task_base, uint32_t NB,
                            const uint32_t* big_list, const uint32_t* big_count, uint32_t S, hipStream_t s) {
    hipLaunchKernelGGL((msm_big_bucket_kernel<P>), dim3(128), dim3(256), 256 * sizeof(Plane29<P>), s, records, cnt, task_start, group_task_base, NB, big_list,
                       big_count, S);
}
#define LURK_FINALIZE_INSTANTIATE(P)                                                                                                                      \
    template void msm_launch_finalize<P>(Plane29<P>*, const uint32_t*, const uint32_t*, const uint32_t*, uint32_t, uint32_t*, uint32_t*, uint32_t, hipStream_t); \
    template void msm_launch_big_buckets<P>(Plane29<P>*, const uint32_t*, const uint32_t*, const uint32_t*, uint32_t, const uint32_t*, const uint32_t*, uint32_t, \
                                            hipStream_t);
#ifdef LURK_MSM_BN254_TU
LURK_FINALIZE_INSTANTIATE(Bn254Fq)
LURK_FINALIZE_INSTANTIATE(Bn254Fr)
#else
LURK_FINALIZE_INSTANTIATE(PallasFp)
LURK_FINALIZE_INSTANTIATE(PallasFq)
#endif

}
```

### lurk_beta_amd/csrc/msm_reduce.hip

```cpp
#include "common.hpp"
#include "msm_core.cuh"
#include "curve29.cuh"

#ifdef LURK_REDUCE_VGPRS
#define LURK_REDUCE_BOUNDS __launch_bounds__(REDUCE_BLOCK, LURK_REDUCE_VGPRS)
#else
#define LURK_REDUCE_BOUNDS __launch_bounds__(REDUCE_BLOCK, 4)
#endif
#ifndef LURK_REDUCE_COMPACT
#define LURK_REDUCE_COMPACT 1
#endif

namespace lurk {

#if defined(LURK_REDUCE_NOADD)
template <class P>
__device__ __forceinline__ void level_add(Xyzz29<P>& r, bool& r_id, const Xyzz29<P>& h, bool h_id) {
#pragma unroll
    for (int i = 0; i < 9; i++) { r.x.l[i] ^= h.x.l[i]; r.y.l[i] ^= h.y.l[i]; r.zz.l[i] ^= h.zz.l[i]; r.zzz.l[i] ^= h.zzz.l[i]; }
    r_id = r_id && h_id;
}
#else
template <class P>
__device__ __forceinline__ void level_add(Xyzz29<P>& r, bool& r_id, const Xyzz29<P>& h, bool h_id) { xyzz29_add<P>(r, r_id, h, h_id); }
#endif

constexpr int REDUCE_BLOCK = 256;


template <class P, bool FIRST, bool LAST>
__global__ LURK_REDUCE_BOUNDS void msm_planes29_kernel(const Plane29<P>* __restrict__ buckets, const Plane29<P>* __restrict__ in,
                                                                      Plane29<P>* __restrict__ out, Xyzz<P>* __restrict__ out_host, int k, int G, uint32_t B) {
    __builtin_amdgcn_s_setprio(3);
    const size_t nseg_out = (size_t)B >> (k + 1);
    const size_t comps_out = (size_t)k + 2, comps_in = (size_t)k + 1;
    const size_t tid = (size_t)blockIdx.x * REDUCE_BLOCK + threadIdx.x;
    if (tid >= (size_t)G * nseg_out * comps_out) return;
#if LURK_REDUCE_COMPACT
    size_t comp, seg, g;
    const size_t adders = (size_t)G * nseg_out * comps_in;
    if (tid < adders) {
        comp = tid % comps_in;
        seg = (tid / comps_in) % nseg_out;
        g = tid / (comps_in * nseg_out);
    } else {
        comp = comps_in;
        seg = (tid - adders) % nseg_out;
        g = (tid - adders) / nseg_out;
    }
    const size_t id = (g * nseg_out + seg) * comps_out + comp;
#else
    const size_t id = tid;
    const size_t comp = id % comps_out, seg = (id / comps_out) % nseg_out, g = id / (comps_out * nseg_out);
#endif
    Xyzz29<P> r, h;
    bool r_id, h_id;
    if (FIRST) {
        plane_load<P>(buckets + (g * B + 2 * seg + 1), h, h_id);
        if (comp == 0) {
            plane_load<P>(buckets + (g * B + 2 * seg), r, r_id);
            level_add<P>(r, r_id, h, h_id);
        } else {
            r = h;
            r_id = h_id;
        }
    } else {
        const Plane29<P>* lo = in + ((g * (nseg_out * 2) + 2 * seg) * comps_in);
        const Plane29<P>* hi = lo + comps_in;
        if (comp <= (size_t)k) {
            plane_load<P>(lo + comp, r, r_id);
            plane_load<P>(hi + comp, h, h_id);
            level_add<P>(r, r_id, h, h_id);
        } else {
            plane_load<P>(hi, r, r_id);
        }
    }
    if (LAST) {
        out_host[id] = xyzz29_to_xyzz<P>(r, r_id);
    } else {
        plane_store<P>(out + id, r, r_id);
    }
}

template <class P, bool FIRST>
__global__ LURK_REDUCE_BOUNDS void msm_planes29_quad_kernel(const Plane29<P>* __restrict__ buckets, const Plane29<P>* __restrict__ in,
                                                                           Plane29<P>* __restrict__ out, int k, int G, uint32_t B) {
    __builtin_amdgcn_s_setprio(3);
    const size_t nseg_out = (size_t)B >> (k + 2);
    const size_t ci = (size_t)k + 1, co = ci + 2;
    const size_t tid = (size_t)blockIdx.x * REDUCE_BLOCK + threadIdx.x;
    const size_t heavy = (size_t)G * nseg_out * ci;
    if (tid >= heavy + (size_t)G * nseg_out) return;
    size_t comp, seg, g;
    const bool light = tid >= heavy;
    if (!light) {
        comp = tid % ci;
        seg = (tid / ci) % nseg_out;
        g = tid / (ci * nseg_out);
    } else {
        comp = 0;
        seg = (tid - heavy) % nseg_out;
        g = (tid - heavy) / nseg_out;
    }
    auto load = [&](int q, Xyzz29<P>& v, bool& id) {
        if (FIRST) {
            plane_load<P>(buckets + (g * B + 4 * seg + q), v, id);
        } else {
            plane_load<P>(in + ((g * (nseg_out * 4) + 4 * seg + q) * ci + comp), v, id);
        }
    };
    auto store = [&](size_t c_out, const Xyzz29<P>& v, bool id) {
        plane_store<P>(out + ((g * nseg_out + seg) * co + c_out), v, id);
    };
    Xyzz29<P> r, h;
    bool r_id, h_id;
    if (light) {
        load(1, r, r_id);
        load(3, h, h_id);
        level_add<P>(r, r_id, h, h_id);
        store(ci, r, r_id);
        return;
    }
    load(2, r, r_id);
    load(3, h, h_id);
    level_add<P>(r, r_id, h, h_id);
    if (comp == 0) store(ci + 1, r, r_id);
    load(0, h, h_id);
    level_add<P>(r, r_id, h, h_id);
    load(1, h, h_id);
    level_add<P>(r, r_id, h, h_id);
    store(comp, r, r_id);
}

template <class P, bool LAST>
__global__ LURK_REDUCE_BOUNDS void msm_planes29_wave_kernel(const Plane29<P>* __restrict__ in, Plane29<P>* __restrict__ out,
                                                                           Xyzz<P>* __restrict__ out_host, int K, int LOG, int G, uint32_t nseg_in) {
    __builtin_amdgcn_s_setprio(3);
    const size_t comps_in = (size_t)K + 1, comps_out = comps_in + LOG;
    const uint32_t lane = threadIdx.x & 63;
    const size_t wave = ((size_t)blockIdx.x * REDUCE_BLOCK + threadIdx.x) >> 6;
    const size_t chunks = ((size_t)nseg_in + 63) / 64;
    if (wave >= (size_t)G * comps_out * chunks) return;
    const size_t chunk = wave % chunks, comp = (wave / chunks) % comps_out, g = wave / (chunks * comps_out);
    const size_t seg = chunk * 64 + lane;
    Xyzz29<P> r;
    bool r_id = true;
#pragma unroll
    for (int i = 0; i < 9; i++) r.x.l[i] = r.y.l[i] = r.zz.l[i] = r.zzz.l[i] = 0;
    if (seg < nseg_in) {
        const Plane29<P>* src = in + (g * nseg_in + seg) * comps_in;
        if (comp < comps_in) plane_load<P>(src + comp, r, r_id);
        else if ((seg >> (comp - comps_in)) & 1) plane_load<P>(src, r, r_id);
    }
    for (int t = 0; t < LOG; t++) {
        const int m = 1 << t;
        Xyzz29<P> h;
#pragma unroll
        for (int i = 0; i < 9; i++) {
            h.x.l[i] = (uint32_t)__shfl_xor((int)r.x.l[i], m);
            h.y.l[i] = (uint32_t)__shfl_xor((int)r.y.l[i], m);
            h.zz.l[i] = (uint32_t)__shfl_xor((int)r.zz.l[i], m);
            h.zzz.l[i] = (uint32_t)__shfl_xor((int)r.zzz.l[i], m);
        }
        const bool h_id = __shfl_xor((int)r_id, m) != 0;
        xyzz29_add<P>(r, r_id, h, h_id);
    }
    if ((lane & ((1u << LOG) - 1u)) != 0 || seg >= nseg_in) return;
    const size_t nseg_out = (size_t)nseg_in >> LOG;
    const size_t id = (g * nseg_out + (seg >> LOG)) * comps_out + comp;
    if (LAST) {
        out_host[id] = xyzz29_to_xyzz<P>(r, r_id);
    } else {
        plane_store<P>(out + id, r, r_id);
    }
}

#ifndef LURK_MSM_BN254_TU
size_t msm_reduce_plane_bytes(size_t nb) { return nb * 160; }
#endif

static bool reduce_wave_levels() {
    static const bool on = [] { const char* v = getenv("LURK_MSM_REDUCE_WAVE"); return !v || atoi(v) != 0; }();
    return on;
}

static bool reduce_quad_levels() {
    static const bool on = [] { const char* v = getenv("LURK_MSM_REDUCE_QUAD"); return !v || atoi(v) != 0; }();
    return on;
}

template <class P>
void msm_launch_reduce(const Plane29<P>* buckets, void* planes_a, void* planes_b, int c, int G, uint32_t B, Xyzz<P>* out_host, hipStream_t s) {
    static_assert(sizeof(Plane29<P>) == 160, "plane record");
    Plane29<P>* bufs[2] = {(Plane29<P>*)planes_a, (Plane29<P>*)planes_b};
    int K = c - 1;
    if (reduce_wave_levels() && c >= 3 && B == (1u << (c - 1))) {
        K = c - 1 > 12 ? c - 1 - 12 : 0;
        if (K < 1) K = 1;
        const size_t cap = (size_t)num_cus() * 4 * 2;
        auto waves = [&](int k) {
            const int rem = c - 1 - k, log1 = rem > 6 ? rem - rem / 2 : rem;
            return (size_t)G * ((((size_t)B >> k) + 63) / 64) * (size_t)(k + 1 + log1);
        };
        while (K < c - 1 && waves(K) > cap) K++;
    }
    const Plane29<P>* src = bufs[1];
    Plane29<P>* dst = bufs[0];
    auto swap = [&] {
        Plane29<P>* t = dst;
        dst = const_cast<Plane29<P>*>(src);
        src = t;
    };
    int k = 0;
    while (k < K) {
        if (reduce_quad_levels() && k + 2 <= K && k + 2 <= c - 2) {
            const size_t threads = (size_t)G * ((size_t)B >> (k + 2)) * (k + 2);
            const dim3 grid(div_up(threads, REDUCE_BLOCK)), block(REDUCE_BLOCK);
            if (k == 0) hipLaunchKernelGGL((msm_planes29_quad_kernel<P, true>), grid, block, 0, s, buckets, src, dst, k, G, B);
            else hipLaunchKernelGGL((msm_planes29_quad_kernel<P, false>), grid, block, 0, s, buckets, src, dst, k, G, B);
            k += 2;
        } else {
            const size_t threads = (size_t)G * ((size_t)B >> (k + 1)) * (k + 2);
            const dim3 grid(div_up(threads, REDUCE_BLOCK)), block(REDUCE_BLOCK);
            const bool last = k == c - 2;
            if (k == 0 && last) hipLaunchKernelGGL((msm_planes29_kernel<P, true, true>), grid, block, 0, s, buckets, src, dst, out_host, k, G, B);
            else if (k == 0) hipLaunchKernelGGL((msm_planes29_kernel<P, true, false>), grid, block, 0, s, buckets, src, dst, out_host, k, G, B);
            else if (last) hipLaunchKernelGGL((msm_planes29_kernel<P, false, true>), grid, block, 0, s, buckets, src, dst, out_host, k, G, B);
            else hipLaunchKernelGGL((msm_planes29_kernel<P, false, false>), grid, block, 0, s, buckets, src, dst, out_host, k, G, B);
            k += 1;
        }
        swap();
    }
    while (k < c - 1) {
        const int rem = c - 1 - k, log = rem > 6 ? rem - rem / 2 : rem;
        const uint32_t nseg_in = B >> k;
        const size_t nwaves = (size_t)G * (((size_t)nseg_in + 63) / 64) * (size_t)(k + 1 + log);
        const dim3 grid(div_up(nwaves * 64, REDUCE_BLOCK)), block(REDUCE_BLOCK);
        if (k + log == c - 1) hipLaunchKernelGGL((msm_planes29_wave_kernel<P, true>), grid, block, 0, s, src, dst, out_host, k, log, G, nseg_in);
        else hipLaunchKernelGGL((msm_planes29_wave_kernel<P, false>), grid, block, 0, s, src, dst, out_host, k, log, G, nseg_in);
        swap();
        k += log;
    }
    LURK_HIP_CHECK(hipGetLastError());
}
#ifdef LURK_MSM_BN254_TU
template void msm_launch_reduce<Bn254Fq>(const Plane29<Bn254Fq>*, void*, void*, int, int, uint32_t, Xyzz<Bn254Fq>*, hipStream_t);
template void msm_launch_reduce<Bn254Fr>(const Plane29<Bn254Fr>*, void*, void*, int, int, uint32_t, Xyzz<Bn254Fr>*, hipStream_t);
#else
template void msm_launch_reduce<PallasFp>(const Plane29<PallasFp>*, void*, void*, int, int, uint32_t, Xyzz<PallasFp>*, hipStream_t);
template void msm_launch_reduce<PallasFq>(const Plane29<PallasFq>*, void*, void*, int, int, uint32_t, Xyzz<PallasFq>*, hipStream_t);
#endif

}
```

### lurk_beta_amd/csrc/msm_sort.hip

```cpp
#include "msm_sort.hpp"

#include "common.hpp"
#include "msm_core.cuh"

namespace lurk {

MsmShape msm_make_shape(int c, bool precomputed, size_t npoints, size_t n, int sel) {
    MsmShape sh;
    sh.c = c;
    sh.W = msm_num_windows(c);
    sh.sel = precomputed ? sel : -1;
    sh.low_prio = 0;
    sh.G = precomputed ? (sh.sel >= 0 ? 2 : 1) : sh.W;
    sh.B = 1u << (c - 1);
    sh.NB = (uint32_t)sh.G * sh.B;
    sh.P = MSM_P_MIN;
    while (sh.P < MSM_P_MAX && (uint32_t)sh.P < sh.NB) {
        int lb = 0;
        while ((sh.NB >> lb) > (uint32_t)sh.P) lb++;
        if (lb <= MSM_LB_MAX && (double)sh.W * (double)n / sh.P <= 0.85 * (double)msm_part2_cap(lb)) break;
        sh.P *= 2;
    }
    sh.LB = 0;
    while ((sh.NB >> sh.LB) > (uint32_t)sh.P) sh.LB++;
    LURK_REQUIRE(sh.LB <= MSM_LB_MAX, "sort shape: more than 8 low key bits per partition");
    sh.tile = MSM_SORT_BLOCK;
    while (sh.tile > 64 && msm_scatter1_lds(sh.P, sh.W, sh.tile) > MSM_LDS_BYTES) sh.tile /= 2;
    sh.S = MSM_S;
    static const size_t task_target = [] { const char* e = getenv("LURK_MSM_TASK_TARGET"); long v = e ? atol(e) : 0; return v > 0 ? (size_t)v : MSM_TASK_TARGET; }();
    while (sh.S > MSM_S_MIN && (size_t)sh.W * n / sh.S < task_target) sh.S /= 2;
    sh.NG = (int)(sh.NB / MSM_GRP);
    sh.n = n;
    sh.stride = precomputed ? npoints : 0;
    return sh;
}

__device__ __forceinline__ void msm_sort_wave_prio(int low = 0) {
    if (low) __builtin_amdgcn_s_setprio(0);
    else __builtin_amdgcn_s_setprio(3);
}

__device__ __forceinline__ uint32_t msm_key(const MsmShape& sh, uint32_t w, uint32_t mag, size_t i) {
    const uint32_t space = sh.sel >= 0 ? (uint32_t)((i >> sh.sel) & 1u) : (sh.G == 1 ? 0u : w);
    return space * sh.B + mag - 1u;
}

constexpr int msm_ct_windows(int C) { return C ? (256 + C - 1) / C : 1; }

template <class SF, int C, bool MONT>
__global__ __launch_bounds__(MSM_SORT_BLOCK) void msm_hist1_kernel(const uint4* __restrict__ scalars, uint4* __restrict__ canon,
                                                                     uint32_t* __restrict__ block_hist, MsmShape sh, size_t chunk) {
    msm_sort_wave_prio(sh.low_prio);
    extern __shared__ uint32_t h[];
    for (int p = threadIdx.x; p < sh.P; p += MSM_SORT_BLOCK) h[p] = 0;
    __syncthreads();
    size_t lo = (size_t)blockIdx.x * chunk, hi = lo + chunk < sh.n ? lo + chunk : sh.n;
    size_t i = lo + threadIdx.x;
    uint4 nlo = make_uint4(0, 0, 0, 0), nhi = nlo;
    if (i < hi) { nlo = scalars[2 * i]; nhi = scalars[2 * i + 1]; }
    for (; i < hi; i += MSM_SORT_BLOCK) {
        Fe<SF> s;
        s.l[0] = nlo.x; s.l[1] = nlo.y; s.l[2] = nlo.z; s.l[3] = nlo.w;
        s.l[4] = nhi.x; s.l[5] = nhi.y; s.l[6] = nhi.z; s.l[7] = nhi.w;
        if (i + MSM_SORT_BLOCK < hi) { nlo = scalars[2 * (i + MSM_SORT_BLOCK)]; nhi = scalars[2 * (i + MSM_SORT_BLOCK) + 1]; }
        if constexpr (MONT) {
            s = fe_from_mont<SF>(s);
            canon[2 * i] = make_uint4(s.l[0], s.l[1], s.l[2], s.l[3]);
            canon[2 * i + 1] = make_uint4(s.l[4], s.l[5], s.l[6], s.l[7]);
        }
        if constexpr (C != 0) {
            uint32_t d[msm_ct_windows(C)];
            msm_digits_ct<C>(s.l, d);
#pragma unroll
            for (int w = 0; w < msm_ct_windows(C); w++) {
                const uint32_t mag = d[w] & ~MSM_SIGN;
                if (mag) atomicAdd(&h[msm_key(sh, (uint32_t)w, mag, i) >> sh.LB], 1u);
            }
        } else {
            uint32_t carry = 0;
            uint32_t r[8];
#pragma unroll
            for (int k = 0; k < 8; k++) r[k] = s.l[k];
            for (int w = 0; w < sh.W; w++) {
                uint32_t mag = msm_digit_next(r, sh.c, carry) & ~MSM_SIGN;
                if (mag) atomicAdd(&h[msm_key(sh, (uint32_t)w, mag, i) >> sh.LB], 1u);
            }
        }
    }
    __syncthreads();
    for (int p = threadIdx.x; p < sh.P; p += MSM_SORT_BLOCK) block_hist[(size_t)blockIdx.x * sh.P + p] = h[p];
}

__global__ __launch_bounds__(MSM_NB1) void msm_scan1_kernel(uint32_t* __restrict__ block_hist, uint32_t* __restrict__ part_cnt, int P) {
    msm_sort_wave_prio();
    __shared__ uint32_t sh[MSM_NB1];
    const int p = blockIdx.x, t = threadIdx.x;
    uint32_t v = block_hist[(size_t)t * P + p];
    sh[t] = v;
    __syncthreads();
    for (int off = 1; off < MSM_NB1; off <<= 1) {
        uint32_t a = t >= off ? sh[t - off] : 0;
        __syncthreads();
        sh[t] += a;
        __syncthreads();
    }
    block_hist[(size_t)t * P + p] = sh[t] - v;
    if (t == MSM_NB1 - 1) part_cnt[p] = sh[t];
}

__device__ __forceinline__ uint32_t msm_block_scan(uint32_t v, uint32_t* scr, uint32_t* total) {
    const int lane = threadIdx.x & 63, wave = threadIdx.x >> 6;
    uint32_t inc = v;
#pragma unroll
    for (int off = 1; off < 64; off <<= 1) {
        uint32_t o = __shfl_up(inc, off);
        if (lane >= off) inc += o;
    }
    if (lane == 63) scr[wave] = inc;
    __syncthreads();
    if (threadIdx.x < 64) {
        uint32_t w = threadIdx.x < MSM_SORT_BLOCK / 64 ? scr[threadIdx.x] : 0, winc = w;
#pragma unroll
        for (int off = 1; off < 16; off <<= 1) {
            uint32_t o = __shfl_up(winc, off);
            if (lane >= off) winc += o;
        }
        if (threadIdx.x < MSM_SORT_BLOCK / 64) scr[threadIdx.x] = winc - w;
        if (threadIdx.x == MSM_SORT_BLOCK / 64 - 1) scr[16] = winc;
    }
    __syncthreads();
    uint32_t ex = scr[wave] + inc - v;
    *total = scr[16];
    __syncthreads();
    return ex;
}

__global__ __launch_bounds__(MSM_SORT_BLOCK) void msm_part_start_kernel(const uint32_t* __restrict__ part_cnt, uint32_t* __restrict__ part_start,
                                                                          int P, uint32_t* __restrict__ z0, int n0, uint32_t* __restrict__ z1, int n1,
                                                                          uint32_t* __restrict__ z2, int n2) {
    msm_sort_wave_prio();
    for (int i = threadIdx.x; i < n0; i += MSM_SORT_BLOCK) z0[i] = 0;
    for (int i = threadIdx.x; i < n1; i += MSM_SORT_BLOCK) z1[i] = 0;
    for (int i = threadIdx.x; i < n2; i += MSM_SORT_BLOCK) z2[i] = 0;
    __shared__ uint32_t scr[32];
    const int PER = P / MSM_SORT_BLOCK;
    const int t = threadIdx.x;
    uint32_t c[MSM_P_PER_MAX], sum = 0;
#pragma unroll
    for (int j = 0; j < MSM_P_PER_MAX; j++) { c[j] = j < PER ? part_cnt[t * PER + j] : 0u; sum += c[j]; }
    uint32_t total;
    uint32_t run = msm_block_scan(sum, scr, &total);
#pragma unroll
    for (int j = 0; j < MSM_P_PER_MAX; j++)
        if (j < PER) { part_start[t * PER + j] = run; run += c[j]; }
    if (t == 0) part_start[P] = total;
}

#ifndef LURK_SORT_MIN_BLOCKS
#define LURK_SORT_MIN_BLOCKS 1
#endif
template <int C>
__global__ __launch_bounds__(MSM_SORT_BLOCK, LURK_SORT_MIN_BLOCKS) void msm_scatter1_kernel(const uint4* __restrict__ scalars, const uint32_t* __restrict__ block_off,
                                                                        const uint32_t* __restrict__ part_start, uint32_t* __restrict__ inter_e,
                                                                        uint8_t* __restrict__ inter_k, MsmShape sh, size_t chunk) {
    msm_sort_wave_prio(sh.low_prio);
    extern __shared__ uint32_t lds[];
    const int P = sh.P, PER = P / MSM_SORT_BLOCK;
    uint32_t* goff = lds;
    uint32_t* cnt = goff + P;
    uint32_t* start = cnt + P;
    uint32_t* scr = start + P;
    uint2* stage = reinterpret_cast<uint2*>(scr + 32);
    const int t = threadIdx.x;
    const uint32_t low_mask = (1u << sh.LB) - 1u;
    for (int p = t; p < P; p += MSM_SORT_BLOCK) {
        goff[p] = part_start[p] + block_off[(size_t)blockIdx.x * P + p];
        cnt[p] = 0;
    }
    __syncthreads();
    size_t lo = (size_t)blockIdx.x * chunk, hi = lo + chunk < sh.n ? lo + chunk : sh.n;
    for (size_t base = lo; base < hi; base += sh.tile) {
        const size_t i = base + t;
        const bool live = t < sh.tile && i < hi;
        uint32_t sl[8];
        uint32_t d[msm_ct_windows(C)];
        if (live) {
            const uint4 a = scalars[2 * i], b = scalars[2 * i + 1];
            sl[0] = a.x; sl[1] = a.y; sl[2] = a.z; sl[3] = a.w;
            sl[4] = b.x; sl[5] = b.y; sl[6] = b.z; sl[7] = b.w;
            if constexpr (C != 0) {
                msm_digits_ct<C>(sl, d);
#pragma unroll
                for (int w = 0; w < msm_ct_windows(C); w++) {
                    const uint32_t mag = d[w] & ~MSM_SIGN;
                    if (mag) atomicAdd(&cnt[msm_key(sh, (uint32_t)w, mag, i) >> sh.LB], 1u);
                }
            } else {
                uint32_t carry = 0;
                uint32_t r[8];
#pragma unroll
                for (int k = 0; k < 8; k++) r[k] = sl[k];
                for (int w = 0; w < sh.W; w++) {
                    uint32_t mag = msm_digit_next(r, sh.c, carry) & ~MSM_SIGN;
                    if (mag) atomicAdd(&cnt[msm_key(sh, (uint32_t)w, mag, i) >> sh.LB], 1u);
                }
            }
        }
        __syncthreads();
        uint32_t total;
        {
            uint32_t c[MSM_P_PER_MAX], sum = 0;
#pragma unroll
            for (int j = 0; j < MSM_P_PER_MAX; j++) { c[j] = j < PER ? cnt[t * PER + j] : 0u; sum += c[j]; }
            uint32_t run = msm_block_scan(sum, scr, &total);
#pragma unroll
            for (int j = 0; j < MSM_P_PER_MAX; j++)
                if (j < PER) { start[t * PER + j] = run; run += c[j]; cnt[t * PER + j] = 0; }
        }
        __syncthreads();
        if (live) {
            if constexpr (C != 0) {
#pragma unroll
                for (int w = 0; w < msm_ct_windows(C); w++) {
                    const uint32_t mag = d[w] & ~MSM_SIGN;
                    if (mag) {
                        const uint32_t key = msm_key(sh, (uint32_t)w, mag, i);
                        const uint32_t p = key >> sh.LB;
                        const uint32_t slot = start[p] + atomicAdd(&cnt[p], 1u);
                        stage[slot] = make_uint2(key, ((uint32_t)((size_t)w * sh.stride) + (uint32_t)i) | (d[w] & MSM_SIGN));
                    }
                }
            } else {
                uint32_t carry = 0;
                uint32_t r[8];
#pragma unroll
                for (int k = 0; k < 8; k++) r[k] = sl[k];
                for (int w = 0; w < sh.W; w++) {
                    uint32_t dg = msm_digit_next(r, sh.c, carry);
                    uint32_t mag = dg & ~MSM_SIGN;
                    if (mag) {
                        uint32_t key = msm_key(sh, (uint32_t)w, mag, i);
                        uint32_t p = key >> sh.LB;
                        uint32_t slot = start[p] + atomicAdd(&cnt[p], 1u);
                        stage[slot] = make_uint2(key, ((uint32_t)((size_t)w * sh.stride) + (uint32_t)i) | (dg & MSM_SIGN));
                    }
                }
            }
        }
        __syncthreads();
        for (uint32_t j = t; j < total; j += MSM_SORT_BLOCK) {
            const uint2 e = stage[j];
            const uint32_t p = e.x >> sh.LB;
            const uint32_t dst = goff[p] + (j - start[p]);
            inter_e[dst] = e.y;
            inter_k[dst] = (uint8_t)(e.x & low_mask);
        }
        __syncthreads();
        for (int j = 0; j < PER; j++) {
            goff[t * PER + j] += cnt[t * PER + j];
            cnt[t * PER + j] = 0;
        }
        __syncthreads();
    }
}

__global__ __launch_bounds__(MSM_SORT_BLOCK) void msm_part2_kernel(const uint32_t* __restrict__ inter_e, const uint8_t* __restrict__ inter_k,
                                                                     const uint32_t* __restrict__ part_start, uint32_t* __restrict__ sorted,
                                                                     uint32_t* __restrict__ cnt, uint32_t* __restrict__ bucket_start, MsmShape sh,
                                                                     uint32_t cap) {
    msm_sort_wave_prio(sh.low_prio);
    extern __shared__ uint32_t lds[];
    const int p = blockIdx.x, t = threadIdx.x;
    const uint32_t nbins = 1u << sh.LB;
    uint32_t* h = lds;
    uint32_t* scr = lds + nbins;
    uint32_t* stage = scr + 32;
    for (uint32_t b = t; b < nbins; b += MSM_SORT_BLOCK) h[b] = 0;
    __syncthreads();
    const uint32_t lo = part_start[p], hi = part_start[p + 1];
    const uint32_t lo4 = lo & ~3u;
    const bool staged = hi - lo <= cap;
    constexpr int U = 4;
    const uint32_t* key_words = reinterpret_cast<const uint32_t*>(inter_k);
    const uint4* entry_quads = reinterpret_cast<const uint4*>(inter_e);
    for (uint32_t base = lo4; base < hi; base += MSM_SORT_BLOCK * 4 * U) {
        uint32_t kw[U];
#pragma unroll
        for (int u = 0; u < U; u++) {
            const uint32_t e = base + (uint32_t)(u * MSM_SORT_BLOCK + t) * 4u;
            kw[u] = e < hi ? key_words[e >> 2] : 0u;
        }
#pragma unroll
        for (int u = 0; u < U; u++) {
            const uint32_t e = base + (uint32_t)(u * MSM_SORT_BLOCK + t) * 4u;
#pragma unroll
            for (int b = 0; b < 4; b++)
                if (e + b >= lo && e + b < hi) atomicAdd(&h[(kw[u] >> (8 * b)) & 0xffu], 1u);
        }
    }
    __syncthreads();
    const uint32_t per = (nbins + MSM_SORT_BLOCK - 1) / MSM_SORT_BLOCK;
    uint32_t sum = 0;
    for (uint32_t j = 0; j < per; j++) {
        uint32_t b = t * per + j;
        if (b < nbins) sum += h[b];
    }
    uint32_t total;
    uint32_t run = lo + msm_block_scan(sum, scr, &total);
    for (uint32_t j = 0; j < per; j++) {
        uint32_t b = t * per + j;
        if (b < nbins) {
            uint32_t c = h[b];
            size_t key = ((size_t)p << sh.LB) + b;
            cnt[key] = c;
            bucket_start[key] = run;
            h[b] = run;
            run += c;
        }
    }
    __syncthreads();
    for (uint32_t base = lo4; base < hi; base += MSM_SORT_BLOCK * 4 * U) {
        uint32_t kw[U];
        uint4 ev[U];
#pragma unroll
        for (int u = 0; u < U; u++) {
            const uint32_t e = base + (uint32_t)(u * MSM_SORT_BLOCK + t) * 4u;
            if (e < hi) { kw[u] = key_words[e >> 2]; ev[u] = entry_quads[e >> 2]; }
            else { kw[u] = 0u; ev[u] = make_uint4(0, 0, 0, 0); }
        }
#pragma unroll
        for (int u = 0; u < U; u++) {
            const uint32_t e = base + (uint32_t)(u * MSM_SORT_BLOCK + t) * 4u;
            const uint32_t ent[4] = {ev[u].x, ev[u].y, ev[u].z, ev[u].w};
#pragma unroll
            for (int b = 0; b < 4; b++) {
                if (e + b >= lo && e + b < hi) {
                    const uint32_t pos = atomicAdd(&h[(kw[u] >> (8 * b)) & 0xffu], 1u);
                    if (staged) stage[pos - lo] = ent[b];
                    else sorted[pos] = ent[b];
                }
            }
        }
    }
    if (staged) {
        __syncthreads();
        for (uint32_t j = t; j < hi - lo; j += MSM_SORT_BLOCK) sorted[lo + j] = stage[j];
    }
}

template <class SF, int C>
static void msm_launch_sort_c(const MsmShape& sh, const void* d_scalars, int is_mont, const MsmSortBufs& b, hipStream_t s) {
    const size_t chunk = (sh.n + MSM_NB1 - 1) / MSM_NB1;
    const size_t entries = (size_t)sh.W * sh.n;
    uint32_t* inter_e = reinterpret_cast<uint32_t*>(b.inter);
    uint8_t* inter_k = reinterpret_cast<uint8_t*>(inter_e + entries);
    allow_dynamic_lds((const void*)msm_scatter1_kernel<C>, (int)MSM_LDS_BYTES);
    allow_dynamic_lds((const void*)msm_part2_kernel, (int)MSM_LDS_BYTES);
    LURK_REQUIRE(msm_scatter1_lds(sh.P, sh.W, sh.tile) <= MSM_LDS_BYTES, "pass-1 tile does not fit the LDS");
    const uint4* canon = (const uint4*)d_scalars;
    if (is_mont) {
        hipLaunchKernelGGL((msm_hist1_kernel<SF, C, true>), dim3(MSM_NB1), dim3(MSM_SORT_BLOCK), (size_t)sh.P * 4, s, (const uint4*)d_scalars,
                           (uint4*)b.canon, b.block_hist, sh, chunk);
        canon = (const uint4*)b.canon;
    } else {
        hipLaunchKernelGGL((msm_hist1_kernel<SF, C, false>), dim3(MSM_NB1), dim3(MSM_SORT_BLOCK), (size_t)sh.P * 4, s, (const uint4*)d_scalars,
                           (uint4*)nullptr, b.block_hist, sh, chunk);
    }
    hipLaunchKernelGGL(msm_scan1_kernel, dim3(sh.P), dim3(MSM_NB1), 0, s, b.block_hist, b.part_cnt, sh.P);
    hipLaunchKernelGGL(msm_part_start_kernel, dim3(1), dim3(MSM_SORT_BLOCK), 0, s, b.part_cnt, b.part_start, sh.P, b.zero[0], b.zero_n[0], b.zero[1],
                       b.zero_n[1], b.zero[2], b.zero_n[2]);
    hipLaunchKernelGGL((msm_scatter1_kernel<C>), dim3(MSM_NB1), dim3(MSM_SORT_BLOCK), msm_scatter1_lds(sh.P, sh.W, sh.tile), s, canon, b.block_hist,
                       b.part_start, inter_e, inter_k, sh, chunk);
    hipLaunchKernelGGL(msm_part2_kernel, dim3(sh.P), dim3(MSM_SORT_BLOCK), MSM_LDS_BYTES, s, inter_e, inter_k, b.part_start, b.sorted, b.cnt,
                       b.bucket_start, sh, (uint32_t)msm_part2_cap(sh.LB));
}

template <class SF>
void msm_launch_sort(const MsmShape& sh, const void* d_scalars, int is_mont, const MsmSortBufs& b, hipStream_t s) {
    if (sh.c == 20) msm_launch_sort_c<SF, 20>(sh, d_scalars, is_mont, b, s);
    else if (sh.c == 16) msm_launch_sort_c<SF, 16>(sh, d_scalars, is_mont, b, s);
    else msm_launch_sort_c<SF, 0>(sh, d_scalars, is_mont, b, s);
}
template void msm_launch_sort<PallasFp>(const MsmShape&, const void*, int, const MsmSortBufs&, hipStream_t);
template void msm_launch_sort<PallasFq>(const MsmShape&, const void*, int, const MsmSortBufs&, hipStream_t);

void msm_launch_sort_canonical(const MsmShape& sh, const void* d_scalars, const MsmSortBufs& b, hipStream_t s) {
    msm_launch_sort<PallasFp>(sh, d_scalars, 0, b, s);
}

}
```

Baseline: 1184.

## Use signed-limb lazy XYZZ additions in bucket sums and add sparse Montgomery exit

```diff
diff --git a/lurk_beta_amd/csrc/common.hpp b/lurk_beta_amd/csrc/common.hpp
--- a/lurk_beta_amd/csrc/common.hpp
+++ b/lurk_beta_amd/csrc/common.hpp
@@ -3,6 +3,7 @@
 
 #include <cstdint>
 #include <cstdio>
+#include <cstdlib>
 #include <cstring>
 #include <condition_variable>
 #include <functional>
@@ -252,6 +253,11 @@
 
 inline unsigned div_up(size_t a, size_t b) { return (unsigned)((a + b - 1) / b); }
 
+inline bool msm_add_signed_enabled() {
+    static const bool on = [] { const char* v = getenv("LURK_MSM_ADD_SIGNED"); return !v || atoi(v) != 0; }();
+    return on;
+}
+
 int num_cus();
 unsigned grid_cap(unsigned per_cu);
 void stream_pool_retain();
diff --git a/lurk_beta_amd/csrc/curve29.cuh b/lurk_beta_amd/csrc/curve29.cuh
--- a/lurk_beta_amd/csrc/curve29.cuh
+++ b/lurk_beta_amd/csrc/curve29.cuh
@@ -422,6 +422,104 @@
     acc.zzz = f29_mul30<P>(zzz12, ppp);
 }
 
+#ifndef LURK_ADD_SIGNED
+#define LURK_ADD_SIGNED 1
+#endif
+template <class P>
+LURK_HD LURK_F29_RARE_ATTR Xyzz29<P> xyzz29_double_general_s(Xyzz29<P> a) {
+    xyzz29_norm_s<P>(a);
+    const Xyzz<P> d = xyzz_dbl<P>(xyzz29_to_xyzz<P>(a, false));
+    Xyzz29<P> r;
+    bool id;
+    xyzz29_from_xyzz<P>(d, r, id);
+    return r;
+}
+template <class P>
+LURK_HD void xyzz29_add_s(Xyzz29<P>& acc, bool& acc_id, const Xyzz29<P>& q, bool q_id) {
+    if (q_id) return;
+    if (acc_id) {
+        acc = q;
+        acc_id = false;
+        return;
+    }
+    F29S_ASSERT_ACC(acc.x, "add_s acc.x"); F29S_ASSERT_ACC(acc.y, "add_s acc.y"); F29S_ASSERT_ACC(acc.zz, "add_s acc.zz"); F29S_ASSERT_ACC(acc.zzz, "add_s acc.zzz");
+    F29S_ASSERT_ACC(q.x, "add_s q.x"); F29S_ASSERT_ACC(q.y, "add_s q.y"); F29S_ASSERT_ACC(q.zz, "add_s q.zz"); F29S_ASSERT_ACC(q.zzz, "add_s q.zzz");
+    const F29<P> u1 = f29_mul_s<P>(acc.x, q.zz);
+    const F29<P> u2 = f29_mul_s<P>(q.x, acc.zz);
+    const F29<P> s1 = f29_mul_s<P>(acc.y, q.zzz);
+    const F29<P> s2 = f29_mul_s<P>(q.y, acc.zzz);
+    const F29<P> p = f29_sub_s<P>(u2, u1);
+    const F29<P> r = f29_sub_s<P>(s2, s1);
+    if (f29_maybe_multiple_of_p_s<P>(p) && f29_is_multiple_of_p_s<P>(p)) {
+        if (f29_maybe_multiple_of_p_s<P>(r) && f29_is_multiple_of_p_s<P>(r)) {
+            acc = xyzz29_double_general_s<P>(acc);
+        } else {
+            acc_id = true;
+        }
+        return;
+    }
+    const F29<P> pp = f29_sqr_s<P>(p);
+    const F29<P> ppp = f29_mul_s<P>(p, pp);
+    const F29<P> qq = f29_mul_s<P>(u1, pp);
+    const F29<P> r2 = f29_sqr_s<P>(r);
+    F29<P> x3;
+#pragma unroll
+    for (int i = 0; i < 9; i++) x3.l[i] = r2.l[i] - ppp.l[i] - (qq.l[i] << 1);
+    x3 = f29_carry_s<P>(x3);
+    const F29<P> d = f29_sub_s<P>(qq, x3);
+    const F29<P> y3 = dot29_row2_s<P>(r, d, f29_neg_s<P>(s1), ppp);
+    const F29<P> zz12 = f29_mul_s<P>(acc.zz, q.zz);
+    const F29<P> zzz12 = f29_mul_s<P>(acc.zzz, q.zzz);
+    acc.x = x3;
+    acc.y = y3;
+    acc.zz = f29_mul_s<P>(zz12, pp);
+    acc.zzz = f29_mul_s<P>(zzz12, ppp);
+    F29S_ASSERT_ACC(acc.x, "add_s acc.x out"); F29S_ASSERT_ACC(acc.y, "add_s acc.y out"); F29S_ASSERT_ACC(acc.zz, "add_s acc.zz out"); F29S_ASSERT_ACC(acc.zzz, "add_s acc.zzz out");
+}
+template <class P>
+LURK_HD constexpr bool msm_add_signed() {
+    return LURK_ADD_SIGNED != 0 && f29_p1_form<P>();
+}
+template <class P, bool SADD>
+LURK_HD void xyzz29_add_sum(Xyzz29<P>& acc, bool& acc_id, const Xyzz29<P>& q, bool q_id) {
+    if constexpr (SADD) xyzz29_add_s<P>(acc, acc_id, q, q_id);
+    else xyzz29_add<P>(acc, acc_id, q, q_id);
+}
+template <class P>
+LURK_HD constexpr uint32_t f29_p16(int i) {
+    uint64_t c = 0;
+    uint32_t limb = 0;
+    for (int k = 0; k <= i; k++) {
+        c += (uint64_t)16 * f29_mod<P>(k);
+        limb = k < 8 ? (uint32_t)c & F29_MASK : (uint32_t)c;
+        c >>= 29;
+    }
+    return limb;
+}
+template <class P>
+LURK_HD F29<P> f29_norm_sum_s(const F29<P>& a) {
+    F29_ASSERT_LIMBS8(a, "f29_norm_sum_s");
+    F29_ASSERT((int32_t)a.l[8] >= -(1 << 26) && (int32_t)a.l[8] < (1 << 27), "f29_norm_sum_s: value outside (-2^258, 2^259)");
+    const uint32_t neg = (uint32_t)((int32_t)a.l[8] >> 31);
+    F29<P> t;
+#pragma unroll
+    for (int i = 0; i < 9; i++) t.l[i] = f29_p16<P>(i) != 0u ? a.l[i] + (neg & f29_p16<P>(i)) : a.l[i];
+    t = f29_carry_s<P>(t);
+    F29_ASSERT_LIMBS(t, 29, "f29_norm_sum_s out"); F29_ASSERT_TOP(t, 27, "f29_norm_sum_s out");
+    return t;
+}
+template <class P, bool SADD>
+LURK_HD void xyzz29_sum_close(Xyzz29<P>& acc, bool acc_id) {
+    if constexpr (SADD) {
+        if (!acc_id) {
+            acc.x = f29_norm_sum_s<P>(acc.x);
+            acc.y = f29_norm_sum_s<P>(acc.y);
+            acc.zz = f29_norm_sum_s<P>(acc.zz);
+            acc.zzz = f29_norm_sum_s<P>(acc.zzz);
+        }
+    }
+}
+
 template <class P>
 LURK_HD Xyzz<P> xyzz_sum_via29(const Xyzz<P>* pts, uint32_t nt) {
     if (nt == 0) return xyzz_identity<P>();
@@ -448,6 +546,14 @@
     id = r.id != 0;
 }
 template <class P>
+LURK_HD void plane_store_raw(Plane29<P>* __restrict__ dst, const Xyzz29<P>& v, bool id) {
+    Plane29<P> o;
+    o.p = v;
+    o.id = id;
+    o.pad[0] = o.pad[1] = o.pad[2] = 0;
+    *dst = o;
+}
+template <class P>
 LURK_HD void plane_store(Plane29<P>* __restrict__ dst, const Xyzz29<P>& v, bool id) {
     if (!id) {
         F29_ASSERT_LIMBS(v.x, 29, "record x"); F29_ASSERT_TOP(v.x, 27, "record x");
@@ -455,11 +561,7 @@
         F29_ASSERT_LIMBS(v.zz, 29, "record zz"); F29_ASSERT_TOP(v.zz, 27, "record zz");
         F29_ASSERT_LIMBS(v.zzz, 29, "record zzz"); F29_ASSERT_TOP(v.zzz, 27, "record zzz");
     }
-    Plane29<P> o;
-    o.p = v;
-    o.id = id;
-    o.pad[0] = o.pad[1] = o.pad[2] = 0;
-    *dst = o;
+    plane_store_raw<P>(dst, v, id);
 }
 template <class P>
 LURK_HD void plane_store_identity(Plane29<P>* __restrict__ dst) {
@@ -467,18 +569,19 @@
     z.x = z.y = z.zz = z.zzz = f29_zero<P>();
     plane_store<P>(dst, z, true);
 }
-template <class P>
+template <class P, bool SADD = msm_add_signed<P>()>
 LURK_HD void plane_sum(const Plane29<P>* recs, uint32_t nt, Xyzz29<P>& acc, bool& acc_id) {
     plane_load<P>(recs, acc, acc_id);
     for (uint32_t i = 1; i < nt; i++) {
         Xyzz29<P> q;
         bool q_id;
         plane_load<P>(recs + i, q, q_id);
-        xyzz29_add<P>(acc, acc_id, q, q_id);
-    }
-}
-
-template <class P>
+        xyzz29_add_sum<P, SADD>(acc, acc_id, q, q_id);
+    }
+    if (nt > 1) xyzz29_sum_close<P, SADD>(acc, acc_id);
+}
+
+template <class P, bool SADD = msm_add_signed<P>()>
 LURK_HD bool plane_finalize_bucket(Plane29<P>* records, uint32_t NB, size_t key, uint32_t nt, uint32_t first, uint32_t fin_small) {
     if (nt == 1) return false;
     if (nt == 0) {
@@ -488,27 +591,28 @@
     if (nt > fin_small) return true;
     Xyzz29<P> acc;
     bool acc_id;
-    plane_sum<P>(records + NB + first, nt, acc, acc_id);
+    plane_sum<P, SADD>(records + NB + first, nt, acc, acc_id);
     plane_store<P>(records + key, acc, acc_id);
     return false;
 }
 
 #if defined(__HIPCC__)
-template <class P, int BLOCK>
+template <class P, int BLOCK, bool SADD = msm_add_signed<P>()>
 __device__ __forceinline__ void block_tree_sum29(Xyzz29<P>& acc, bool& acc_id, Plane29<P>* sh) {
     const int t = threadIdx.x;
-    plane_store<P>(sh + t, acc, acc_id);
+    plane_store_raw<P>(sh + t, acc, acc_id);
     __syncthreads();
     for (int stride = BLOCK / 2; stride >= 1; stride >>= 1) {
         if (t < stride) {
             Xyzz29<P> q;
             bool q_id;
             plane_load<P>(sh + t + stride, q, q_id);
-            xyzz29_add<P>(acc, acc_id, q, q_id);
-            plane_store<P>(sh + t, acc, acc_id);
+            xyzz29_add_sum<P, SADD>(acc, acc_id, q, q_id);
+            plane_store_raw<P>(sh + t, acc, acc_id);
         }
         __syncthreads();
     }
+    if (t == 0) xyzz29_sum_close<P, SADD>(acc, acc_id);
 }
 #endif
 
diff --git a/lurk_beta_amd/csrc/field.cuh b/lurk_beta_amd/csrc/field.cuh
--- a/lurk_beta_amd/csrc/field.cuh
+++ b/lurk_beta_amd/csrc/field.cuh
@@ -516,6 +516,47 @@
     return fe_mul<P>(a, one);
 }
 template <class P>
+LURK_HD constexpr bool fe_exit_sparse() {
+    return P::mod(0) == 1u && P::INV == 0xffffffffu;
+}
+template <class P>
+LURK_HD Fe<P> fe_exit_mont(const Fe<P>& a) {
+    uint32_t t[8];
+#pragma unroll
+    for (int i = 0; i < 8; i++) t[i] = a.l[i];
+#pragma unroll
+    for (int k = 0; k < 8; k++) {
+        const uint32_t m = fe_exit_sparse<P>() ? 0u - t[0] : t[0] * P::INV;
+        uint32_t lo[8], hi[8];
+#pragma unroll
+        for (int j = 0; j < 8; j++) {
+            if (j == 0 && fe_exit_sparse<P>()) {
+                lo[j] = m;
+                hi[j] = 0;
+            } else if (P::mod(j) != 0u) {
+                const uint64_t x = (uint64_t)m * P::mod(j);
+                lo[j] = (uint32_t)x;
+                hi[j] = (uint32_t)(x >> 32);
+            } else {
+                lo[j] = hi[j] = 0;
+            }
+        }
+        uint32_t w[9], cy = 0;
+#pragma unroll
+        for (int j = 1; j < 8; j++) w[j] = addc32(lo[j], hi[j - 1], cy);
+        w[8] = hi[7] + cy;
+        uint32_t c = t[0] != 0u ? 1u : 0u;
+#pragma unroll
+        for (int j = 1; j < 8; j++) t[j - 1] = addc32(t[j], w[j], c);
+        t[7] = w[8] + c;
+    }
+    fe_cond_sub<P>(t);
+    Fe<P> r;
+#pragma unroll
+    for (int i = 0; i < 8; i++) r.l[i] = t[i];
+    return r;
+}
+template <class P>
 LURK_HD Fe<P> fe_from_u64(uint64_t v) {
     Fe<P> x = fe_zero<P>();
     x.l[0] = (uint32_t)v;
diff --git a/lurk_beta_amd/csrc/msm_batch.hip b/lurk_beta_amd/csrc/msm_batch.hip
--- a/lurk_beta_amd/csrc/msm_batch.hip
+++ b/lurk_beta_amd/csrc/msm_batch.hip
@@ -53,7 +53,7 @@
         Fe<SF> s;
         s.l[0] = lo4.x; s.l[1] = lo4.y; s.l[2] = lo4.z; s.l[3] = lo4.w;
         s.l[4] = hi4.x; s.l[5] = hi4.y; s.l[6] = hi4.z; s.l[7] = hi4.w;
-        if (is_mont) s = fe_from_mont<SF>(s);
+        if (is_mont) s = fe_exit_mont<SF>(s);
 #pragma unroll
         for (int t = 0; t < 8; t++) s8[t] = s.l[t];
     }
diff --git a/lurk_beta_amd/csrc/msm_bucket_direct.hip b/lurk_beta_amd/csrc/msm_bucket_direct.hip
--- a/lurk_beta_amd/csrc/msm_bucket_direct.hip
+++ b/lurk_beta_amd/csrc/msm_bucket_direct.hip
@@ -4,6 +4,19 @@
 #include "msm_stages.hpp"
 
 namespace lurk {
+
+int msm_bucket_direct_lanes(size_t NB, size_t entries);
+
+#ifdef LURK_MSM_ADDU_TU
+namespace addu {
+static constexpr bool ADDU_TU = true;
+#else
+static constexpr bool ADDU_TU = false;
+#endif
+template <class P>
+static constexpr bool tu_sadd() {
+    return !ADDU_TU && msm_add_signed<P>();
+}
 
 constexpr int DIRECT_BLOCK = 256;
 constexpr uint32_t DIRECT_CAP = 64;
@@ -14,6 +27,7 @@
                                                                            uint32_t NB, Plane29<P>* __restrict__ buckets, uint32_t* __restrict__ big_list,
                                                                            uint32_t* __restrict__ big_count) {
     __builtin_amdgcn_s_setprio(1);
+    constexpr bool SADD = tu_sadd<P>();
     const size_t lane = (size_t)blockIdx.x * DIRECT_BLOCK + threadIdx.x;
     size_t key = lane / L;
     const uint32_t sub = (uint32_t)(lane % L);
@@ -45,8 +59,9 @@
             o.zzz.l[k] = __shfl_xor(acc.zzz.l[k], off);
         }
         o_id = __shfl_xor((int)acc_id, off) != 0;
-        xyzz29_add<P>(acc, acc_id, o, o_id);
+        xyzz29_add_sum<P, SADD>(acc, acc_id, o, o_id);
     }
+    if (L > 1) xyzz29_sum_close<P, SADD>(acc, acc_id);
     if (live && !big && sub == 0) plane_store<P>(buckets + key, acc, acc_id);
 }
 
@@ -68,13 +83,13 @@
             const uint32_t e = sorted[start + j];
             xyzz29_madd<P>(acc, acc_id, table[e & 0x7fffffffu], (e & 0x80000000u) != 0);
         }
-        block_tree_sum29<P, DIRECT_BLOCK>(acc, acc_id, sh);
+        block_tree_sum29<P, DIRECT_BLOCK, tu_sadd<P>()>(acc, acc_id, sh);
         if (threadIdx.x == 0) plane_store<P>(buckets + key, acc, acc_id);
         __syncthreads();
     }
 }
 
-#ifndef LURK_MSM_BN254_TU
+#if !defined(LURK_MSM_BN254_TU) && !defined(LURK_MSM_ADDU_TU)
 int msm_bucket_direct_lanes(size_t NB, size_t entries) {
     int L = 1;
     while (L < 4 && NB * (size_t)(2 * L) <= 131072 && entries / (NB * (size_t)(2 * L)) >= 4) L *= 2;
@@ -82,9 +97,20 @@
 }
 #endif
 
+#if !defined(LURK_MSM_ADDU_TU) && !defined(LURK_MSM_BN254_TU) && LURK_ADD_SIGNED && LURK_F29_P1
+#define LURK_HAVE_ADDU 1
+namespace addu {
+template <class P>
+void msm_launch_bucket_direct(const uint32_t* sorted, const Affine<P>* table, const uint32_t* bucket_start, const uint32_t* cnt, uint32_t NB, size_t entries,
+                              Plane29<P>* buckets, uint32_t* big_list, uint32_t* big_count, hipStream_t s);
+}
+#endif
 template <class P>
 void msm_launch_bucket_direct(const uint32_t* sorted, const Affine<P>* table, const uint32_t* bucket_start, const uint32_t* cnt, uint32_t NB, size_t entries,
                               Plane29<P>* buckets, uint32_t* big_list, uint32_t* big_count, hipStream_t s) {
+#ifdef LURK_HAVE_ADDU
+    if (!msm_add_signed_enabled()) return addu::msm_launch_bucket_direct<P>(sorted, table, bucket_start, cnt, NB, entries, buckets, big_list, big_count, s);
+#endif
     const int L = msm_bucket_direct_lanes(NB, entries);
     const dim3 grid((unsigned)div_up((size_t)NB * L, DIRECT_BLOCK)), block(DIRECT_BLOCK);
     if (L == 1) hipLaunchKernelGGL((msm_bucket_direct_kernel<P, 1>), grid, block, 0, s, sorted, table, bucket_start, cnt, NB, buckets, big_list, big_count);
@@ -96,7 +122,12 @@
 #define LURK_DIRECT_INSTANTIATE(P)                                                                                                                      \
     template void msm_launch_bucket_direct<P>(const uint32_t*, const Affine<P>*, const uint32_t*, const uint32_t*, uint32_t, size_t, Plane29<P>*, uint32_t*, \
                                               uint32_t*, hipStream_t);
-#ifdef LURK_MSM_BN254_TU
+#if defined(LURK_MSM_ADDU_TU)
+#if LURK_ADD_SIGNED && LURK_F29_P1
+LURK_DIRECT_INSTANTIATE(PallasFp)
+LURK_DIRECT_INSTANTIATE(PallasFq)
+#endif
+#elif defined(LURK_MSM_BN254_TU)
 LURK_DIRECT_INSTANTIATE(Bn254Fq)
 LURK_DIRECT_INSTANTIATE(Bn254Fr)
 #else
@@ -104,4 +135,8 @@
 LURK_DIRECT_INSTANTIATE(PallasFq)
 #endif
 
+#ifdef LURK_MSM_ADDU_TU
 }
+#endif
+
+}
diff --git a/lurk_beta_amd/csrc/msm_bucket_direct_addu.hip b/lurk_beta_amd/csrc/msm_bucket_direct_addu.hip
--- /dev/null
+++ b/lurk_beta_amd/csrc/msm_bucket_direct_addu.hip
@@ -0,0 +1,2 @@
+#define LURK_MSM_ADDU_TU 1
+#include "msm_bucket_direct.hip"
diff --git a/lurk_beta_amd/csrc/msm_finalize.hip b/lurk_beta_amd/csrc/msm_finalize.hip
--- a/lurk_beta_amd/csrc/msm_finalize.hip
+++ b/lurk_beta_amd/csrc/msm_finalize.hip
@@ -4,6 +4,17 @@
 #include "msm_stages.hpp"
 
 namespace lurk {
+
+#ifdef LURK_MSM_ADDU_TU
+namespace addu {
+static constexpr bool ADDU_TU = true;
+#else
+static constexpr bool ADDU_TU = false;
+#endif
+template <class P>
+static constexpr bool tu_sadd() {
+    return !ADDU_TU && msm_add_signed<P>();
+}
 
 #ifndef LURK_FINALIZE_WAVES
 #define LURK_FINALIZE_WAVES 4
@@ -22,7 +33,7 @@
         const uint32_t g = (uint32_t)(key / MSM_GRP), b = (uint32_t)(key % MSM_GRP);
         first = group_task_base[g] + task_start[(size_t)g * (MSM_GRP + 1) + b];
     }
-    if (plane_finalize_bucket<P>(records, NB, key, nt, first, MSM_FIN_SMALL)) big_list[atomicAdd(big_count, 1u)] = (uint32_t)key;
+    if (plane_finalize_bucket<P, tu_sadd<P>()>(records, NB, key, nt, first, MSM_FIN_SMALL)) big_list[atomicAdd(big_count, 1u)] = (uint32_t)key;
 }
 
 template <class P>
@@ -30,6 +41,7 @@
                                                                const uint32_t* __restrict__ group_task_base, uint32_t NB,
                                                                const uint32_t* __restrict__ big_list, const uint32_t* __restrict__ big_count, uint32_t S) {
     __builtin_amdgcn_s_setprio(3);
+    constexpr bool SADD = tu_sadd<P>();
     extern __shared__ uint4 lds_raw[];
     Plane29<P>* sh = reinterpret_cast<Plane29<P>*>(lds_raw);
     const uint32_t nbig = *big_count;
@@ -43,24 +55,41 @@
         bool acc_id = true, q_id;
         for (uint32_t j = threadIdx.x; j < nt; j += 256) {
             plane_load<P>(tasks + j, q, q_id);
-            xyzz29_add<P>(acc, acc_id, q, q_id);
+            xyzz29_add_sum<P, SADD>(acc, acc_id, q, q_id);
         }
-        block_tree_sum29<P, 256>(acc, acc_id, sh);
+        block_tree_sum29<P, 256, SADD>(acc, acc_id, sh);
         if (threadIdx.x == 0) plane_store<P>(records + key, acc, acc_id);
         __syncthreads();
     }
 }
 
+#if !defined(LURK_MSM_ADDU_TU) && !defined(LURK_MSM_BN254_TU) && LURK_ADD_SIGNED && LURK_F29_P1
+#define LURK_HAVE_ADDU 1
+namespace addu {
+template <class P>
+void msm_launch_finalize(Plane29<P>* records, const uint32_t* cnt, const uint32_t* task_start, const uint32_t* group_task_base, uint32_t NB,
+                         uint32_t* big_list, uint32_t* big_count, uint32_t S, hipStream_t s);
+template <class P>
+void msm_launch_big_buckets(Plane29<P>* records, const uint32_t* cnt, const uint32_t* task_start, const uint32_t* group_task_base, uint32_t NB,
+                            const uint32_t* big_list, const uint32_t* big_count, uint32_t S, hipStream_t s);
+}
+#endif
 template <class P>
 void msm_launch_finalize(Plane29<P>* records, const uint32_t* cnt, const uint32_t* task_start, const uint32_t* group_task_base, uint32_t NB,
                          uint32_t* big_list, uint32_t* big_count, uint32_t S, hipStream_t s) {
     static_assert(sizeof(Plane29<P>) == MSM_RECORD_BYTES, "the slot's record array is sized by MSM_RECORD_BYTES");
+#ifdef LURK_HAVE_ADDU
+    if (!msm_add_signed_enabled()) return addu::msm_launch_finalize<P>(records, cnt, task_start, group_task_base, NB, big_list, big_count, S, s);
+#endif
     hipLaunchKernelGGL((msm_finalize_kernel<P>), dim3(div_up((size_t)NB, 256)), dim3(256), 0, s, records, cnt, task_start, group_task_base, NB, big_list, big_count,
                        S);
 }
 template <class P>
 void msm_launch_big_buckets(Plane29<P>* records, const uint32_t* cnt, const uint32_t* task_start, const uint32_t* group_task_base, uint32_t NB,
                             const uint32_t* big_list, const uint32_t* big_count, uint32_t S, hipStream_t s) {
+#ifdef LURK_HAVE_ADDU
+    if (!msm_add_signed_enabled()) return addu::msm_launch_big_buckets<P>(records, cnt, task_start, group_task_base, NB, big_list, big_count, S, s);
+#endif
     hipLaunchKernelGGL((msm_big_bucket_kernel<P>), dim3(128), dim3(256), 256 * sizeof(Plane29<P>), s, records, cnt, task_start, group_task_base, NB, big_list,
                        big_count, S);
 }
@@ -68,7 +97,12 @@
     template void msm_launch_finalize<P>(Plane29<P>*, const uint32_t*, const uint32_t*, const uint32_t*, uint32_t, uint32_t*, uint32_t*, uint32_t, hipStream_t); \
     template void msm_launch_big_buckets<P>(Plane29<P>*, const uint32_t*, const uint32_t*, const uint32_t*, uint32_t, const uint32_t*, const uint32_t*, uint32_t, \
                                             hipStream_t);
-#ifdef LURK_MSM_BN254_TU
+#if defined(LURK_MSM_ADDU_TU)
+#if LURK_ADD_SIGNED && LURK_F29_P1
+LURK_FINALIZE_INSTANTIATE(PallasFp)
+LURK_FINALIZE_INSTANTIATE(PallasFq)
+#endif
+#elif defined(LURK_MSM_BN254_TU)
 LURK_FINALIZE_INSTANTIATE(Bn254Fq)
 LURK_FINALIZE_INSTANTIATE(Bn254Fr)
 #else
@@ -76,4 +110,8 @@
 LURK_FINALIZE_INSTANTIATE(PallasFq)
 #endif
 
+#ifdef LURK_MSM_ADDU_TU
 }
+#endif
+
+}
diff --git a/lurk_beta_amd/csrc/msm_finalize_addu.hip b/lurk_beta_amd/csrc/msm_finalize_addu.hip
--- /dev/null
+++ b/lurk_beta_amd/csrc/msm_finalize_addu.hip
@@ -0,0 +1,2 @@
+#define LURK_MSM_ADDU_TU 1
+#include "msm_finalize.hip"
diff --git a/lurk_beta_amd/csrc/msm_reduce.hip b/lurk_beta_amd/csrc/msm_reduce.hip
--- a/lurk_beta_amd/csrc/msm_reduce.hip
+++ b/lurk_beta_amd/csrc/msm_reduce.hip
@@ -13,17 +13,31 @@
 
 namespace lurk {
 
+#ifdef LURK_MSM_ADDU_TU
+namespace addu {
+static constexpr bool ADDU_TU = true;
+#else
+static constexpr bool ADDU_TU = false;
+#endif
+template <class P>
+static constexpr bool tu_sadd() {
+    return !ADDU_TU && msm_add_signed<P>();
+}
+
 #if defined(LURK_REDUCE_NOADD)
-template <class P>
+template <class P, bool SADD>
 __device__ __forceinline__ void level_add(Xyzz29<P>& r, bool& r_id, const Xyzz29<P>& h, bool h_id) {
 #pragma unroll
     for (int i = 0; i < 9; i++) { r.x.l[i] ^= h.x.l[i]; r.y.l[i] ^= h.y.l[i]; r.zz.l[i] ^= h.zz.l[i]; r.zzz.l[i] ^= h.zzz.l[i]; }
     r_id = r_id && h_id;
 }
 #else
-template <class P>
-__device__ __forceinline__ void level_add(Xyzz29<P>& r, bool& r_id, const Xyzz29<P>& h, bool h_id) { xyzz29_add<P>(r, r_id, h, h_id); }
-#endif
+template <class P, bool SADD>
+__device__ __forceinline__ void level_add(Xyzz29<P>& r, bool& r_id, const Xyzz29<P>& h, bool h_id) { xyzz29_add_sum<P, SADD>(r, r_id, h, h_id); }
+#endif
+
+template <class P, bool SADD>
+__device__ __forceinline__ void level_close(Xyzz29<P>& r, bool r_id) { xyzz29_sum_close<P, SADD>(r, r_id); }
 
 constexpr int REDUCE_BLOCK = 256;
 
@@ -32,6 +46,7 @@
 __global__ LURK_REDUCE_BOUNDS void msm_planes29_kernel(const Plane29<P>* __restrict__ buckets, const Plane29<P>* __restrict__ in,
                                                                       Plane29<P>* __restrict__ out, Xyzz<P>* __restrict__ out_host, int k, int G, uint32_t B) {
     __builtin_amdgcn_s_setprio(3);
+    constexpr bool SADD = tu_sadd<P>();
     const size_t nseg_out = (size_t)B >> (k + 1);
     const size_t comps_out = (size_t)k + 2, comps_in = (size_t)k + 1;
     const size_t tid = (size_t)blockIdx.x * REDUCE_BLOCK + threadIdx.x;
@@ -59,7 +74,8 @@
         plane_load<P>(buckets + (g * B + 2 * seg + 1), h, h_id);
         if (comp == 0) {
             plane_load<P>(buckets + (g * B + 2 * seg), r, r_id);
-            level_add<P>(r, r_id, h, h_id);
+            level_add<P, SADD>(r, r_id, h, h_id);
+            level_close<P, SADD>(r, r_id);
         } else {
             r = h;
             r_id = h_id;
@@ -70,7 +86,8 @@
         if (comp <= (size_t)k) {
             plane_load<P>(lo + comp, r, r_id);
             plane_load<P>(hi + comp, h, h_id);
-            level_add<P>(r, r_id, h, h_id);
+            level_add<P, SADD>(r, r_id, h, h_id);
+            level_close<P, SADD>(r, r_id);
         } else {
             plane_load<P>(hi, r, r_id);
         }
@@ -86,6 +103,7 @@
 __global__ LURK_REDUCE_BOUNDS void msm_planes29_quad_kernel(const Plane29<P>* __restrict__ buckets, const Plane29<P>* __restrict__ in,
                                                                            Plane29<P>* __restrict__ out, int k, int G, uint32_t B) {
     __builtin_amdgcn_s_setprio(3);
+    constexpr bool SADD = tu_sadd<P>();
     const size_t nseg_out = (size_t)B >> (k + 2);
     const size_t ci = (size_t)k + 1, co = ci + 2;
     const size_t tid = (size_t)blockIdx.x * REDUCE_BLOCK + threadIdx.x;
@@ -117,18 +135,24 @@
     if (light) {
         load(1, r, r_id);
         load(3, h, h_id);
-        level_add<P>(r, r_id, h, h_id);
+        level_add<P, SADD>(r, r_id, h, h_id);
+        level_close<P, SADD>(r, r_id);
         store(ci, r, r_id);
         return;
     }
     load(2, r, r_id);
     load(3, h, h_id);
-    level_add<P>(r, r_id, h, h_id);
-    if (comp == 0) store(ci + 1, r, r_id);
+    level_add<P, SADD>(r, r_id, h, h_id);
+    if (comp == 0) {
+        Xyzz29<P> w = r;
+        level_close<P, SADD>(w, r_id);
+        store(ci + 1, w, r_id);
+    }
     load(0, h, h_id);
-    level_add<P>(r, r_id, h, h_id);
+    level_add<P, SADD>(r, r_id, h, h_id);
     load(1, h, h_id);
-    level_add<P>(r, r_id, h, h_id);
+    level_add<P, SADD>(r, r_id, h, h_id);
+    level_close<P, SADD>(r, r_id);
     store(comp, r, r_id);
 }
 
@@ -136,6 +160,7 @@
 __global__ LURK_REDUCE_BOUNDS void msm_planes29_wave_kernel(const Plane29<P>* __restrict__ in, Plane29<P>* __restrict__ out,
                                                                            Xyzz<P>* __restrict__ out_host, int K, int LOG, int G, uint32_t nseg_in) {
     __builtin_amdgcn_s_setprio(3);
+    constexpr bool SADD = LAST && tu_sadd<P>();
     const size_t comps_in = (size_t)K + 1, comps_out = comps_in + LOG;
     const uint32_t lane = threadIdx.x & 63;
     const size_t wave = ((size_t)blockIdx.x * REDUCE_BLOCK + threadIdx.x) >> 6;
@@ -163,9 +188,10 @@
             h.zzz.l[i] = (uint32_t)__shfl_xor((int)r.zzz.l[i], m);
         }
         const bool h_id = __shfl_xor((int)r_id, m) != 0;
-        xyzz29_add<P>(r, r_id, h, h_id);
+        level_add<P, SADD>(r, r_id, h, h_id);
     }
     if ((lane & ((1u << LOG) - 1u)) != 0 || seg >= nseg_in) return;
+    if (SADD && !r_id) xyzz29_norm_s<P>(r);
     const size_t nseg_out = (size_t)nseg_in >> LOG;
     const size_t id = (g * nseg_out + (seg >> LOG)) * comps_out + comp;
     if (LAST) {
@@ -175,7 +201,7 @@
     }
 }
 
-#ifndef LURK_MSM_BN254_TU
+#if !defined(LURK_MSM_BN254_TU) && !defined(LURK_MSM_ADDU_TU)
 size_t msm_reduce_plane_bytes(size_t nb) { return nb * 160; }
 #endif
 
@@ -189,8 +215,18 @@
     return on;
 }
 
+#if !defined(LURK_MSM_ADDU_TU) && !defined(LURK_MSM_BN254_TU) && LURK_ADD_SIGNED && LURK_F29_P1
+#define LURK_HAVE_ADDU 1
+namespace addu {
+template <class P>
+void msm_launch_reduce(const Plane29<P>* buckets, void* planes_a, void* planes_b, int c, int G, uint32_t B, Xyzz<P>* out_host, hipStream_t s);
+}
+#endif
 template <class P>
 void msm_launch_reduce(const Plane29<P>* buckets, void* planes_a, void* planes_b, int c, int G, uint32_t B, Xyzz<P>* out_host, hipStream_t s) {
+#ifdef LURK_HAVE_ADDU
+    if (!msm_add_signed_enabled()) return addu::msm_launch_reduce<P>(buckets, planes_a, planes_b, c, G, B, out_host, s);
+#endif
     static_assert(sizeof(Plane29<P>) == 160, "plane record");
     Plane29<P>* bufs[2] = {(Plane29<P>*)planes_a, (Plane29<P>*)planes_b};
     int K = c - 1;
@@ -243,7 +279,12 @@
     }
     LURK_HIP_CHECK(hipGetLastError());
 }
-#ifdef LURK_MSM_BN254_TU
+#if defined(LURK_MSM_ADDU_TU)
+#if LURK_ADD_SIGNED && LURK_F29_P1
+template void msm_launch_reduce<PallasFp>(const Plane29<PallasFp>*, void*, void*, int, int, uint32_t, Xyzz<PallasFp>*, hipStream_t);
+template void msm_launch_reduce<PallasFq>(const Plane29<PallasFq>*, void*, void*, int, int, uint32_t, Xyzz<PallasFq>*, hipStream_t);
+#endif
+#elif defined(LURK_MSM_BN254_TU)
 template void msm_launch_reduce<Bn254Fq>(const Plane29<Bn254Fq>*, void*, void*, int, int, uint32_t, Xyzz<Bn254Fq>*, hipStream_t);
 template void msm_launch_reduce<Bn254Fr>(const Plane29<Bn254Fr>*, void*, void*, int, int, uint32_t, Xyzz<Bn254Fr>*, hipStream_t);
 #else
@@ -251,4 +292,8 @@
 template void msm_launch_reduce<PallasFq>(const Plane29<PallasFq>*, void*, void*, int, int, uint32_t, Xyzz<PallasFq>*, hipStream_t);
 #endif
 
-}
+#ifdef LURK_MSM_ADDU_TU
+}
+#endif
+
+}
diff --git a/lurk_beta_amd/csrc/msm_reduce_addu.hip b/lurk_beta_amd/csrc/msm_reduce_addu.hip
--- /dev/null
+++ b/lurk_beta_amd/csrc/msm_reduce_addu.hip
@@ -0,0 +1,2 @@
+#define LURK_MSM_ADDU_TU 1
+#include "msm_reduce.hip"
diff --git a/lurk_beta_amd/csrc/msm_sort.hip b/lurk_beta_amd/csrc/msm_sort.hip
--- a/lurk_beta_amd/csrc/msm_sort.hip
+++ b/lurk_beta_amd/csrc/msm_sort.hip
@@ -64,7 +64,7 @@
         s.l[4] = nhi.x; s.l[5] = nhi.y; s.l[6] = nhi.z; s.l[7] = nhi.w;
         if (i + MSM_SORT_BLOCK < hi) { nlo = scalars[2 * (i + MSM_SORT_BLOCK)]; nhi = scalars[2 * (i + MSM_SORT_BLOCK) + 1]; }
         if constexpr (MONT) {
-            s = fe_from_mont<SF>(s);
+            s = fe_exit_mont<SF>(s);
             canon[2 * i] = make_uint4(s.l[0], s.l[1], s.l[2], s.l[3]);
             canon[2 * i + 1] = make_uint4(s.l[4], s.l[5], s.l[6], s.l[7]);
         }
```

Measured after the change: 1183. About the same (-0.1%).
